# CPCLAB-UNIPI/MPC-code

Measured on NVIDIA B200. Metric: batched MPC steps/sec (Ex_NMPC CSTR, N=50, FP64), higher is better.
Workload: dtype f64

## Files before the change

mpc-code_b200/csrc/mpcb_api.cu:

```cuda
#include <cuda_runtime.h>
#include <stdio.h>
#include <string.h>
#include <stdlib.h>
#include <string>
#include <utility>
#include <vector>
#include "mpcb.h"
#include "mpcb_target.cuh"

#define MPCB_NKERNELS 8
enum { KC_OCP_INIT = 0, KC_OCP_EVAL = 1, KC_OCP_KKT = 2, KC_OCP_TRIAL = 3, KC_OCP_ACCEPT = 4, KC_TARGET = 5, KC_ESTIMATE = 6, KC_OTHER = 7 };

#ifndef MPCB_EVAL_BLOCK
#define MPCB_EVAL_BLOCK 128
#endif
#ifndef MPCB_EVAL_MINBLOCKS
#define MPCB_EVAL_MINBLOCKS 2
#endif

#ifndef MPCB_FLOPS_TABLE
#define MPCB_FLOPS_TABLE
#endif

#if MPCB_HAS_OCP
struct OcpArgs {
    int B;
    const double* par; double* w; double* ws; InstState* st;
    unsigned long long* counters;
    OcpShared S;
};

__device__ __forceinline__ OcpInst ocp_view(const OcpArgs& a, int inst) {
    return ocp_inst(a.ws + (size_t)inst * OcpLayout::total, a.w + (size_t)inst * NW, a.par + (size_t)inst * NPAR, a.st + inst);
}

__global__ void __launch_bounds__(128) k_ocp_init(OcpArgs a) {
    const int tid = blockIdx.x * blockDim.x + threadIdx.x;
    const int inst = tid / (NH + 1), k = tid % (NH + 1);
    if (inst >= a.B) return;
    OcpInst I = ocp_view(a, inst);
    ocp_init_stage(I, a.S, k);
}

#ifndef MPCB_EVAL_SMEM
#define MPCB_EVAL_SMEM ((EVAL_RK_DOUBLES) > 0 && \
                        ((size_t)(EVAL_RK_DOUBLES) * 8 * MPCB_EVAL_BLOCK + 1024) * MPCB_EVAL_MINBLOCKS <= 232448)
#endif
#define EVAL_SMEM_BYTES (MPCB_EVAL_SMEM ? (size_t)(EVAL_RK_DOUBLES) * 8 * MPCB_EVAL_BLOCK : 0)
#ifdef MPCB_EVAL_MAXNREG
#define EVAL_BOUNDS __maxnreg__(MPCB_EVAL_MAXNREG)
#else
#define EVAL_BOUNDS __launch_bounds__(MPCB_EVAL_BLOCK, MPCB_EVAL_MINBLOCKS)
#endif
__global__ void EVAL_BOUNDS k_ocp_eval(OcpArgs a) {
    extern __shared__ double eval_smem[];
    const int tid = blockIdx.x * blockDim.x + threadIdx.x;
    const int inst = tid / NH, k = tid % NH;
    if (inst >= a.B) return;
    if (a.st[inst].state != ST_EVAL) return;
    if (k == 0) atomicAdd(a.counters, 1ULL);
    OcpInst I = ocp_view(a, inst);
    ocp_eval_stage<MPCB_EVAL_SMEM>(I, a.S, k, RkBuf{eval_smem + threadIdx.x, MPCB_EVAL_BLOCK});
}

#if MPCB_EVAL_FIRST
__global__ void __launch_bounds__(128) k_ocp_eval_first(OcpArgs a) {
    const int tid = blockIdx.x * blockDim.x + threadIdx.x;
    const int inst = tid / NH, k = tid % NH;
    if (inst >= a.B) return;
    if (a.st[inst].state != ST_EVAL) return;
    if (k == 0) atomicAdd(a.counters, 1ULL);
    OcpInst I = ocp_view(a, inst);
    ocp_eval_stage<false, true>(I, a.S, k);
}
#endif

#ifndef MPCB_TGT_BLOCK
#define MPCB_TGT_BLOCK 64
#endif
#ifndef KKT_WARPS
#define KKT_SCRATCH_BYTES ((int)sizeof(double) * KktScratch::total * (32 / MPCB_KKT_LANES))
#define KKT_WARPS (4 * KKT_SCRATCH_BYTES <= 48 * 1024 ? 4 : (2 * KKT_SCRATCH_BYTES <= 48 * 1024 ? 2 : 1))
#endif
#if MPCB_KKT_LANES > 1
#ifndef MPCB_FUSE_LS
#define MPCB_FUSE_LS 0
#endif
#ifdef MPCB_KKT_MINBLOCKS
#define KKT_BOUNDS __launch_bounds__(32 * KKT_WARPS, MPCB_KKT_MINBLOCKS)
#else
#define KKT_BOUNDS __launch_bounds__(32 * KKT_WARPS)
#endif
__global__ void KKT_BOUNDS k_ocp_kkt(OcpArgs a, int* n_active) {
    constexpr int GROUPS = 32 * KKT_WARPS / MPCB_KKT_LANES;
    __shared__ __align__(16) double scratch[GROUPS][KktScratch::total];
    const int inst = (blockIdx.x * blockDim.x + threadIdx.x) / MPCB_KKT_LANES;
    if (inst >= a.B) return;
    if (a.st[inst].state != ST_EVAL) return;
    OcpInst I = ocp_view(a, inst);
    ocp_kkt(I, a.S, scratch[threadIdx.x / MPCB_KKT_LANES]);
#if MPCB_FUSE_LS
    const int lane = threadIdx.x & 31;
    volatile int* state = &a.st[inst].state;
    while (*state == ST_LS) {
        if (lane == 0) atomicAdd(a.counters + 1, 1ULL);
        for (int k = lane; k < NH; k += 32) ocp_trial_stage(I, a.S, k);
        __syncwarp();
        ocp_accept(I, a.S);
    }
    if (n_active && lane == 0 && *state != ST_DONE) atomicAdd(n_active, 1);
#else
    (void)n_active;
#endif
}
#define KKT_GRID(B) nblk((long)(B) * MPCB_KKT_LANES, 32 * KKT_WARPS), 32 * KKT_WARPS
#else
#define MPCB_FUSE_LS 0
__global__ void __launch_bounds__(32) k_ocp_kkt(OcpArgs a, int* n_active) {
    (void)n_active;
    const int inst = blockIdx.x * blockDim.x + threadIdx.x;
    if (inst >= a.B) return;
    if (a.st[inst].state != ST_EVAL) return;
    double scratch[KktScratch::total];
    OcpInst I = ocp_view(a, inst);
    ocp_kkt(I, a.S, scratch);
}
#define KKT_GRID(B) nblk((long)(B), 32), 32
#endif

__global__ void __launch_bounds__(128) k_ocp_trial(OcpArgs a) {
    const int tid = blockIdx.x * blockDim.x + threadIdx.x;
    const int inst = tid / NH, k = tid % NH;
    if (inst >= a.B) return;
    if (a.st[inst].state != ST_LS) return;
    if (k == 0) atomicAdd(a.counters + 1, 1ULL);
    OcpInst I = ocp_view(a, inst);
    ocp_trial_stage(I, a.S, k);
}

__global__ void __launch_bounds__(32 * KKT_WARPS) k_ocp_accept(OcpArgs a, int* n_active) {
    const int inst = (blockIdx.x * blockDim.x + threadIdx.x) >> 5;
    if (inst >= a.B) return;
    if (a.st[inst].state == ST_LS) {
        OcpInst I = ocp_view(a, inst);
        ocp_accept(I, a.S);
    }
    if (n_active && (threadIdx.x & 31) == 0 && a.st[inst].state != ST_DONE) atomicAdd(n_active, 1);
}

__global__ void k_ocp_cond(cudaGraphConditionalHandle handle, int* n_active, unsigned long long* ctr, int max_ticks, int ticks) {
    const int active = *n_active;
    *n_active = 0;
    const unsigned long long t = (ctr[0] += (unsigned long long)ticks);
    ctr[1] += (unsigned long long)ticks;
    cudaGraphSetConditional(handle, (active > 0 && t < (unsigned long long)max_ticks) ? 1u : 0u);
}

__global__ void k_ocp_output(OcpArgs a, double* f, int* status, int* iters) {
    const int tid = blockIdx.x * blockDim.x + threadIdx.x;
    const int inst = tid / (NH + 1), k = tid % (NH + 1);
    if (inst >= a.B) return;
    OcpInst I = ocp_view(a, inst);
    ocp_export_stage(I, k);
    if (k == 0) { f[inst] = a.st[inst].fval; status[inst] = a.st[inst].status; iters[inst] = a.st[inst].iter; }
}

__global__ void EVAL_BOUNDS k_stage_derivs(int B, const double* par, const double* w, const double* lam,
                                                      double* A, double* Bm, double* c, double* H) {
    extern __shared__ double eval_smem[];
    const int tid = blockIdx.x * blockDim.x + threadIdx.x;
    const int inst = tid / NH, k = tid % NH;
    if (inst >= B) return;
    const double* wi = w + (size_t)inst * NW; const double* pi = par + (size_t)inst * NPAR;
    double x[NX], u[NU], l[NX], d[ND + 1], px[NPX + 1], py[NPY + 1], t0;
    for (int i = 0; i < NX; ++i) { x[i] = wi[k * NZ + i]; l[i] = lam[((size_t)inst * NH + k) * NX + i]; }
    for (int i = 0; i < NU; ++i) u[i] = wi[k * NZ + NX + i];
    stage_params(pi, k, d, px, py, &t0);
    double xn[NX], Al[NX * NX], Bl[NX * NU], Hp[NZP];
    for (int i = 0; i < NZP; ++i) Hp[i] = 0.0;
    dyn_full<(MPCB_EVAL_SMEM && MPCB_DYN_RK4 && !MPCB_CONTFORM)>(x, u, d, px, t0, l, xn, Al, Bl, Hp, RkBuf{eval_smem + threadIdx.x, MPCB_EVAL_BLOCK});
    const size_t s = (size_t)inst * NH + k;
    for (int i = 0; i < NX * NX; ++i) A[s * NX * NX + i] = Al[i];
    for (int i = 0; i < NX * NU; ++i) Bm[s * NX * NU + i] = Bl[i];
    for (int i = 0; i < NX; ++i) c[s * NX + i] = xn[i] - wi[(k + 1) * NZ + i];
    for (int i = 0; i < NZP; ++i) H[s * NZP + i] = Hp[i];
}
#endif

#if MPCB_HAS_TARGET
__global__ void __launch_bounds__(64) k_target(int B, const double* par, double* w, double* f, int* status, int* iters,
                                               TgtShared S) {
    const int inst = blockIdx.x * blockDim.x + threadIdx.x;
    if (inst >= B) return;
    tgt_solve_regular(par + (size_t)inst * MPCB_NPARSS, w + (size_t)inst * NWS, f + inst, status + inst, iters + inst, S);
}
__global__ void __launch_bounds__(64) k_target_resto(int B, const double* par, double* w, double* f, int* status, int* iters,
                                                     TgtShared S) {
    const int inst = blockIdx.x * blockDim.x + threadIdx.x;
    if (inst >= B) return;
    tgt_solve_resto(par + (size_t)inst * MPCB_NPARSS, w + (size_t)inst * NWS, f + inst, status + inst, iters + inst, S);
}
#endif

__global__ void __launch_bounds__(64) k_estimate(int B, int est_type, const double* y, const double* u, const double* t,
                                                 const double* px, const double* py, double* xi, double* P, EstShared E) {
    const int inst = blockIdx.x * blockDim.x + threadIdx.x;
    if (inst >= B) return;
    est_update(est_type, y + (size_t)inst * NY, u + (size_t)inst * NU, t[inst], px + (size_t)inst * NPX,
               py + (size_t)inst * NPY, xi + (size_t)inst * NXI, P + (size_t)inst * NXI * NXI, E);
}

__global__ void k_model_output(int B, const double* x, const double* u, const double* d, const double* t,
                               const double* py, double* y) {
    const int inst = blockIdx.x * blockDim.x + threadIdx.x;
    if (inst >= B) return;
    double xl[NX], ul[NU], dl[ND + 1], pl[NPY + 1], yl[NY], tt = t[inst];
    for (int i = 0; i < NX; ++i) xl[i] = x[(size_t)inst * NX + i];
    for (int i = 0; i < NU; ++i) ul[i] = u[(size_t)inst * NU + i];
    for (int i = 0; i < ND; ++i) dl[i] = d[(size_t)inst * ND + i];
    for (int i = 0; i < NPY; ++i) pl[i] = py[(size_t)inst * NPY + i];
    mdl_fy(xl, ul, dl, &tt, pl, yl);
    for (int i = 0; i < NY; ++i) y[(size_t)inst * NY + i] = yl[i];
}

__global__ void k_model_step(int B, const double* x, const double* u, const double* d, const double* t,
                             const double* px, double* xn) {
    const int inst = blockIdx.x * blockDim.x + threadIdx.x;
    if (inst >= B) return;
    double xl[NX], ul[NU], dl[ND + 1], pl[NPX + 1], xo[NX];
    for (int i = 0; i < NX; ++i) xl[i] = x[(size_t)inst * NX + i];
    for (int i = 0; i < NU; ++i) ul[i] = u[(size_t)inst * NU + i];
    for (int i = 0; i < ND; ++i) dl[i] = d[(size_t)inst * ND + i];
    for (int i = 0; i < NPX; ++i) pl[i] = px[(size_t)inst * NPX + i];
    dyn_value(xl, ul, dl, pl, t[inst], xo);
    for (int i = 0; i < NX; ++i) xn[(size_t)inst * NX + i] = xo[i];
}

#if !MPCB_PLANT_NOMINAL
__global__ void k_plant_meas(int B, const double* x, const double* u, const double* t, const double* pyp,
                             const double* pymp, const double* noise, double* y) {
    const int inst = blockIdx.x * blockDim.x + threadIdx.x;
    if (inst >= B) return;
    double yl[NY];
    plant_meas(x + (size_t)inst * MPCB_NXP, u + (size_t)inst * NU, t[inst], pyp + (size_t)inst * MPCB_NPYP,
               pymp + (size_t)inst * MPCB_NPYP, yl);
    for (int i = 0; i < NY; ++i) y[(size_t)inst * NY + i] = yl[i] + (noise ? noise[(size_t)inst * NY + i] : 0.0);
}
__global__ void k_plant_step(int B, double* x, const double* u, const double* t, const double* pxp, const double* pxmp) {
    const int inst = blockIdx.x * blockDim.x + threadIdx.x;
    if (inst >= B) return;
    plant_step(x + (size_t)inst * MPCB_NXP, u + (size_t)inst * NU, t[inst], pxp + (size_t)inst * MPCB_NPXP,
               pxmp + (size_t)inst * MPCB_NPXP);
}
#endif


#if MPCB_HAS_OCP && MPCB_HAS_TARGET
struct LoopState {
    double *xi, *P, *u, *us, *xs, *wguess, *wopt, *x0m, *u0, *parss, *wss, *par, *w, *px0, *py0, *fss;
    int *dyn_status, *ss_status, *ss_iters;
};

__global__ void k_step_params(int B, const double* px, const double* py, LoopState L) {
    const int inst = blockIdx.x * blockDim.x + threadIdx.x;
    if (inst >= B) return;
    for (int i = 0; i < NPX; ++i) L.px0[(size_t)inst * NPX + i] = px ? px[(size_t)inst * NPX * NH + i] : 0.0;
    for (int i = 0; i < NPY; ++i) L.py0[(size_t)inst * NPY + i] = py ? py[(size_t)inst * NPY * NH + i] : 0.0;
}

__global__ void k_step_pre(int B, const double* t, const double* sp, LoopState L, double* xhat_out, double* dhat_out) {
    const int inst = blockIdx.x * blockDim.x + threadIdx.x;
    if (inst >= B) return;
    const double* xi = L.xi + (size_t)inst * NXI;
    double* ps = L.parss + (size_t)inst * MPCB_NPARSS;
    for (int i = 0; i < NX; ++i) xhat_out[(size_t)inst * NX + i] = xi[i];
    double d[ND + 1];
    for (int i = 0; i < ND; ++i) { d[i] = (NXI > NX) ? xi[NX + i] : 0.0; dhat_out[(size_t)inst * ND + i] = d[i]; }
    const double* spi = sp + (size_t)inst * (NU + NY + NX);
    for (int i = 0; i < NU; ++i) ps[MPCB_OFFSS_USP + i] = spi[i];
    for (int i = 0; i < NY; ++i) ps[MPCB_OFFSS_YSP + i] = spi[NU + i];
    for (int i = 0; i < NX; ++i) ps[MPCB_OFFSS_XSP + i] = spi[NU + NY + i];
    for (int i = 0; i < ND; ++i) ps[MPCB_OFFSS_D + i] = d[i];
    for (int i = 0; i < NU; ++i) ps[MPCB_OFFSS_USPREV + i] = L.us[(size_t)inst * NU + i];
    for (int i = 0; i < NY * NU; ++i) ps[MPCB_OFFSS_LAM + i] = 0.0;
    ps[MPCB_OFFSS_T] = t[inst];
    double py[NPY + 1];
    for (int i = 0; i < NPX; ++i) ps[MPCB_OFFSS_PX + i] = L.px0[(size_t)inst * NPX + i];
    for (int i = 0; i < NPY; ++i) { py[i] = L.py0[(size_t)inst * NPY + i]; ps[MPCB_OFFSS_PY + i] = py[i]; }
    double* wg = L.wss + (size_t)inst * NWS;
    double x0[NX], u0[NU], y0[NY], tt = t[inst];
    for (int i = 0; i < NX; ++i) { x0[i] = L.x0m[(size_t)inst * NX + i]; wg[i] = x0[i]; }
    for (int i = 0; i < NU; ++i) { u0[i] = L.u0[(size_t)inst * NU + i]; wg[NX + i] = u0[i]; }
    mdl_fy(x0, u0, d, &tt, py, y0);
    for (int i = 0; i < NY; ++i) wg[NZ + i] = y0[i];
}

__global__ void k_step_mid(int B, int first, const double* t, const double* px, const double* py, LoopState L,
                           double* xs_out, double* us_out) {
    const int inst = (blockIdx.x * blockDim.x + threadIdx.x) >> 5, lane = threadIdx.x & 31;
    if (inst >= B) return;
    double* xs = L.xs + (size_t)inst * NX; double* us = L.us + (size_t)inst * NU;
    const double* wss = L.wss + (size_t)inst * NWS;
    const bool ss_ok = L.ss_status[inst] != 2;
    double xs_prev[NX], us_prev[NU], xs_new[NX], us_new[NU];
    for (int i = 0; i < NX; ++i) { xs_prev[i] = xs[i]; xs_new[i] = ss_ok ? wss[i] : xs_prev[i]; }
    for (int i = 0; i < NU; ++i) { us_prev[i] = us[i]; us_new[i] = ss_ok ? wss[NX + i] : us_prev[i]; }
    __syncwarp();
    const double* xi = L.xi + (size_t)inst * NXI;
    double* pr = L.par + (size_t)inst * NPAR;
    if (lane == 0) {
        for (int i = 0; i < NX; ++i) { xs[i] = xs_new[i]; xs_out[(size_t)inst * NX + i] = xs_new[i]; }
        for (int i = 0; i < NU; ++i) { us[i] = us_new[i]; us_out[(size_t)inst * NU + i] = us_new[i]; }
        for (int i = 0; i < NX; ++i) { pr[MPCB_OFF_X0 + i] = xi[i]; pr[MPCB_OFF_XS + i] = xs_new[i]; }
        for (int i = 0; i < NU; ++i) { pr[MPCB_OFF_US + i] = us_new[i]; pr[MPCB_OFF_UM1 + i] = L.u[(size_t)inst * NU + i]; }
        for (int i = 0; i < ND; ++i) pr[MPCB_OFF_D + i] = (NXI > NX) ? xi[NX + i] : 0.0;
        pr[MPCB_OFF_T] = t[inst];
        for (int i = 0; i < NY * NU; ++i) pr[MPCB_OFF_LAM + i] = 0.0;
    }
    for (int i = lane; i < NPX * NH; i += 32) pr[MPCB_OFF_PX + i] = px ? px[(size_t)inst * NPX * NH + i] : 0.0;
    for (int i = lane; i < NPY * NH; i += 32) pr[MPCB_OFF_PY + i] = py ? py[(size_t)inst * NPY * NH + i] : 0.0;
    double* wg = L.wguess + (size_t)inst * NW; double* w = L.w + (size_t)inst * NW;
    const double* wo = L.wopt + (size_t)inst * NW;
    const bool shift = !first && L.dyn_status[inst] != 2 && L.dyn_status[inst] != -13;
    for (int i = lane; i < NW; i += 32) {
        double v;
        if (first) {
            const int r = i % NZ;
            v = (r < NX) ? L.x0m[(size_t)inst * NX + r] : L.u0[(size_t)inst * NU + r - NX];
        } else if (shift) {
            if (i < NW - NZ) v = wo[NZ + i];
            else {
                v = 0.0;
#pragma unroll
                for (int j = 0; j < NU; ++j) if (i == NW - NZ + j) v = us_prev[j];
#pragma unroll
                for (int j = 0; j < NX; ++j) if (i == NW - NX + j) v = xs_prev[j];
            }
        } else {
            v = wg[i];
        }
        wg[i] = v; w[i] = v;
    }
}

__global__ void k_step_post(int B, const double* t, const int* status, LoopState L, double* u_out, int hold_failed) {
    const int inst = (blockIdx.x * blockDim.x + threadIdx.x) >> 5, lane = threadIdx.x & 31;
    if (inst >= B) return;
    double* xi = L.xi + (size_t)inst * NXI; double* u = L.u + (size_t)inst * NU;
    const double* w = L.w + (size_t)inst * NW;
    int st = status[inst];
    if (hold_failed && st < 0 && st != -13) st = 2;
    if (lane == 0) L.dyn_status[inst] = st;
    if (st == -13) {
        for (int i = lane; i < NU; i += 32) u_out[(size_t)inst * NU + i] = u[i];
    } else if (st != 2) {
        double* wo = L.wopt + (size_t)inst * NW;
        for (int i = lane; i < NW; i += 32) wo[i] = w[i];
        for (int i = lane; i < NU; i += 32) { const double v = w[NX + i]; u[i] = v; u_out[(size_t)inst * NU + i] = v; }
        for (int i = lane; i < NX; i += 32) xi[i] = w[NZ + i];
    } else if (lane == 0) {
        double x[NX], ul[NU], d[ND + 1], pxl[NPX + 1], xn[NX];
        for (int i = 0; i < NX; ++i) x[i] = xi[i];
        for (int i = 0; i < NU; ++i) { ul[i] = u[i]; u_out[(size_t)inst * NU + i] = ul[i]; }
        for (int i = 0; i < ND; ++i) d[i] = (NXI > NX) ? xi[NX + i] : 0.0;
        for (int i = 0; i < NPX; ++i) pxl[i] = L.px0[(size_t)inst * NPX + i];
        dyn_value(x, ul, d, pxl, t[inst], xn);
        for (int i = 0; i < NX; ++i) xi[i] = xn[i];
    }
}
#endif

struct mpcb_ctx {
    int B, device;
    mpcb_opts_t opts_ss, opts_dyn;
    std::string err;
    double *ws, *lbx, *ubx, *lbg, *ubg, *ss_lbx, *ss_ubx, *Qkf, *Rkf, *Kest, *dmin, *dmax;
    InstState* st;
    int* n_active; int* h_active;
    int have_dbounds, last_launches, last_ticks;
    cudaGraph_t og_graph; cudaGraphExec_t og_exec;
    const void* og_key[5]; mpcb_opts_t og_opts; int og_valid;
    double* stage_mem; int* stage_imem;
    unsigned long long* tick_ctr;
    long host_launches; int host_loop; cudaStream_t last_stream;
    int hold_failed;
    double* loop_mem; int* loop_imem; int loop_first;
#if MPCB_HAS_OCP && MPCB_HAS_TARGET
    LoopState L;
#endif
    int profile;
    unsigned long long* counters;
    double kernel_ms[MPCB_NKERNELS]; long kernel_launches[MPCB_NKERNELS];
    unsigned long long eval_instances, trial_instances;
    std::vector<cudaEvent_t> ev_pool;
    std::vector<std::pair<int, int>> ev_pending;
    int ngroups;
    std::vector<struct StepGroup*> groups;
    cudaEvent_t ev_in;
};

struct StepGroup { mpcb_ctx* c; int b0, nb; cudaStream_t s; cudaEvent_t done; };

static IpmOpts to_ipm(const mpcb_opts_t& o) {
    IpmOpts r;
    r.max_iter = o.max_iter; r.tol = o.tol; r.mu_init = o.mu_init; r.bound_relax = o.bound_relax_factor;
    r.bound_push = o.bound_push; r.acceptable_tol = o.acceptable_tol;
    r.honor_original_bounds = o.honor_original_bounds; r.acceptable_iter = o.acceptable_iter;
    return r;
}

static int fail(mpcb_ctx* h, const char* what, cudaError_t e) {
    if (h) h->err = std::string(what) + ": " + cudaGetErrorString(e);
    return -1;
}
#define CK(call) do { cudaError_t e_ = (call); if (e_ != cudaSuccess) return fail(h, #call, e_); } while (0)

struct Prof {
    mpcb_ctx* h; cudaStream_t s; int kc; int idx;
    Prof(mpcb_ctx* h_, cudaStream_t s_, int kc_) : h(h_), s(s_), kc(kc_), idx(-1) {
        if (!h->profile) return;
        idx = (int)h->ev_pending.size() * 2;
        while ((int)h->ev_pool.size() < idx + 2) { cudaEvent_t e; cudaEventCreate(&e); h->ev_pool.push_back(e); }
        cudaEventRecord(h->ev_pool[idx], s);
    }
    ~Prof() {
        h->kernel_launches[kc] += 1;
        if (idx < 0) return;
        cudaEventRecord(h->ev_pool[idx + 1], s);
        h->ev_pending.push_back(std::make_pair(kc, idx));
    }
};
static void prof_collect(mpcb_ctx* h) {
    for (auto& p : h->ev_pending) {
        float ms = 0.f;
        if (cudaEventElapsedTime(&ms, h->ev_pool[p.second], h->ev_pool[p.second + 1]) == cudaSuccess) h->kernel_ms[p.first] += ms;
    }
    h->ev_pending.clear();
}

__global__ void k_dfma_peak(double* out, int iters) {
    double a0 = threadIdx.x * 1e-9, a1 = a0 + 1, a2 = a0 + 2, a3 = a0 + 3, a4 = a0 + 4, a5 = a0 + 5, a6 = a0 + 6, a7 = a0 + 7;
    const double b = 1.0000001, c = 1e-9;
    for (int i = 0; i < iters; ++i) {
        a0 = fma(a0, b, c); a1 = fma(a1, b, c); a2 = fma(a2, b, c); a3 = fma(a3, b, c);
        a4 = fma(a4, b, c); a5 = fma(a5, b, c); a6 = fma(a6, b, c); a7 = fma(a7, b, c);
    }
    out[blockIdx.x * blockDim.x + threadIdx.x] = a0 + a1 + a2 + a3 + a4 + a5 + a6 + a7;
}

extern "C" {

int mpcb_abi_version(void) { return MPCB_ABI_VERSION; }

void mpcb_default_opts(mpcb_opts_t* o) {
    o->max_iter = 100; o->tol = 1e-8; o->mu_init = 0.1; o->bound_relax_factor = 1e-8;
    o->honor_original_bounds = 0; o->bound_push = 1e-2; o->acceptable_tol = 1e-6; o->acceptable_iter = 15;
}

int mpcb_get_dims(mpcb_dims_t* d) {
    memset(d, 0, sizeof(*d));
    d->nx = NX; d->nu = NU; d->ny = NY; d->nd = ND; d->npx = NPX; d->npy = NPY;
    d->nxp = MPCB_NXP; d->npxp = MPCB_NPXP; d->npyp = MPCB_NPYP; d->nxi = NXI; d->N = NH; d->Mx = MX;
#if MPCB_HAS_OCP
    d->nw = NW; d->npar = NPAR; d->ng = NG; d->has_ocp = 1;
#endif
#if MPCB_HAS_TARGET
    d->nwss = NWS; d->nparss = MPCB_NPARSS; d->has_target = 1;
#endif
    return 0;
}

long mpcb_model_flops(const char* name) {
    static const struct { const char* n; long f; } table[] = { MPCB_FLOPS_TABLE {nullptr, 0} };
    for (int i = 0; table[i].n; ++i) if (!strcmp(table[i].n, name)) return table[i].f;
    return -1;
}

int mpcb_create(int batch, const mpcb_opts_t* oss, const mpcb_opts_t* odyn, mpcb_handle_t* out) {
    mpcb_ctx* h = new mpcb_ctx();
    h->B = batch; h->have_dbounds = 0; h->last_launches = 0; h->last_ticks = 0;
    h->og_graph = nullptr; h->og_exec = nullptr; h->og_valid = 0; h->tick_ctr = nullptr; h->host_launches = 0; h->last_stream = nullptr;
    h->stage_mem = nullptr; h->stage_imem = nullptr; h->hold_failed = 0;
    { const char* e = getenv("MPCB_HOST_LOOP"); h->host_loop = (e && e[0] == '1') ? 1 : 0; }
    mpcb_default_opts(&h->opts_ss); mpcb_default_opts(&h->opts_dyn);
    if (oss) h->opts_ss = *oss;
    if (odyn) h->opts_dyn = *odyn;
    *out = h;
    if (batch <= 0) { h->err = "batch must be positive"; return -2; }
    CK(cudaGetDevice(&h->device));
    h->ws = nullptr; h->st = nullptr; h->lbx = h->ubx = h->lbg = h->ubg = nullptr;
#if MPCB_HAS_OCP
    CK(cudaMalloc(&h->ws, sizeof(double) * (size_t)batch * OcpLayout::total));
    CK(cudaMemset(h->ws, 0, sizeof(double) * (size_t)batch * OcpLayout::total));
    CK(cudaMalloc(&h->st, sizeof(InstState) * (size_t)batch));
    CK(cudaMalloc(&h->lbx, sizeof(double) * NWI)); CK(cudaMalloc(&h->ubx, sizeof(double) * NWI));
    CK(cudaMalloc(&h->lbg, sizeof(double) * (NH * NGS))); CK(cudaMalloc(&h->ubg, sizeof(double) * (NH * NGS)));
    if (EVAL_SMEM_BYTES > 0) {
        CK(cudaFuncSetAttribute(k_ocp_eval, cudaFuncAttributeMaxDynamicSharedMemorySize, (int)EVAL_SMEM_BYTES));
        CK(cudaFuncSetAttribute(k_stage_derivs, cudaFuncAttributeMaxDynamicSharedMemorySize, (int)EVAL_SMEM_BYTES));
    }
#endif
    h->ss_lbx = h->ss_ubx = nullptr;
#if MPCB_HAS_TARGET
    CK(cudaMalloc(&h->ss_lbx, sizeof(double) * NWS)); CK(cudaMalloc(&h->ss_ubx, sizeof(double) * NWS));
#endif
    CK(cudaMalloc(&h->Qkf, sizeof(double) * NXI * NXI)); CK(cudaMalloc(&h->Rkf, sizeof(double) * NY * NY));
    CK(cudaMalloc(&h->Kest, sizeof(double) * NXI * NY));
    CK(cudaMalloc(&h->dmin, sizeof(double) * (ND + 1))); CK(cudaMalloc(&h->dmax, sizeof(double) * (ND + 1)));
    CK(cudaMemset(h->Qkf, 0, sizeof(double) * NXI * NXI)); CK(cudaMemset(h->Rkf, 0, sizeof(double) * NY * NY));
    CK(cudaMemset(h->Kest, 0, sizeof(double) * NXI * NY));
    CK(cudaMalloc(&h->n_active, sizeof(int)));
    CK(cudaMemset(h->n_active, 0, sizeof(int)));
    CK(cudaMallocHost(&h->h_active, sizeof(int)));
    CK(cudaMalloc(&h->tick_ctr, 2 * sizeof(unsigned long long)));
    CK(cudaMemset(h->tick_ctr, 0, 2 * sizeof(unsigned long long)));
    CK(cudaMalloc(&h->counters, 2 * sizeof(unsigned long long)));
    CK(cudaMemset(h->counters, 0, 2 * sizeof(unsigned long long)));
    h->loop_mem = nullptr; h->loop_imem = nullptr; h->loop_first = 1;
    h->profile = 0; h->eval_instances = h->trial_instances = 0;
    h->ngroups = 1; h->ev_in = nullptr;
    for (int i = 0; i < MPCB_NKERNELS; ++i) { h->kernel_ms[i] = 0.0; h->kernel_launches[i] = 0; }
    return 0;
}

static void groups_teardown(mpcb_ctx* h);

static void ocp_graph_drop(mpcb_ctx* h) {
    if (h->og_exec) cudaGraphExecDestroy(h->og_exec);
    if (h->og_graph) cudaGraphDestroy(h->og_graph);
    h->og_exec = nullptr; h->og_graph = nullptr; h->og_valid = 0;
}

int mpcb_destroy(mpcb_handle_t h) {
    if (!h) return 0;
    cudaDeviceSynchronize();
    groups_teardown(h);
    ocp_graph_drop(h);
    cudaFree(h->tick_ctr); cudaFree(h->stage_mem); cudaFree(h->stage_imem);
    if (h->ev_in) cudaEventDestroy(h->ev_in);
    cudaFree(h->ws); cudaFree(h->st); cudaFree(h->lbx); cudaFree(h->ubx); cudaFree(h->lbg); cudaFree(h->ubg);
    cudaFree(h->ss_lbx); cudaFree(h->ss_ubx); cudaFree(h->Qkf); cudaFree(h->Rkf); cudaFree(h->Kest);
    cudaFree(h->dmin); cudaFree(h->dmax); cudaFree(h->n_active); cudaFreeHost(h->h_active); cudaFree(h->counters);
    for (auto e : h->ev_pool) cudaEventDestroy(e);
    cudaFree(h->loop_mem); cudaFree(h->loop_imem);
    delete h;
    return 0;
}

const char* mpcb_last_error(mpcb_handle_t h) { return h ? h->err.c_str() : "null handle"; }

int mpcb_set_const(mpcb_handle_t h, const char* name, const double* p, int n) {
#if MPCB_HAS_OCP
    if (!strcmp(name, "ocp_lbx") || !strcmp(name, "ocp_ubx")) {
        if (n != NW) { h->err = std::string("mpcb_set_const: wrong length for ") + name; return -2; }
        const bool lower = !strcmp(name, "ocp_lbx");
        std::vector<double> tmp(NWI, lower ? -INFINITY : INFINITY);
        for (int k = 0; k <= NH; ++k) {
            for (int i = 0; i < NX; ++i) tmp[k * NZA + i] = p[k * NZ + i];
            if (k < NH) for (int i = 0; i < NU; ++i) tmp[k * NZA + NXA + i] = p[k * NZ + NX + i];
        }
        CK(cudaMemcpy(lower ? h->lbx : h->ubx, tmp.data(), sizeof(double) * NWI, cudaMemcpyHostToDevice));
        return 0;
    }
#endif
    struct { const char* nm; double* dst; int len; } tab[] = {
#if MPCB_HAS_OCP
        {"ocp_lbg", h->lbg, NH * NG}, {"ocp_ubg", h->ubg, NH * NG},
#endif
#if MPCB_HAS_TARGET
        {"ss_lbx", h->ss_lbx, NWS}, {"ss_ubx", h->ss_ubx, NWS},
#endif
        {"Q_kf", h->Qkf, NXI * NXI}, {"R_kf", h->Rkf, NY * NY}, {"K_est", h->Kest, NXI * NY},
        {"dmin", h->dmin, ND}, {"dmax", h->dmax, ND},
    };
    for (auto& e : tab) {
        if (strcmp(e.nm, name)) continue;
        if (n != e.len) { h->err = std::string("mpcb_set_const: wrong length for ") + name; return -2; }
        if (n > 0) CK(cudaMemcpy(e.dst, p, sizeof(double) * n, cudaMemcpyHostToDevice));
        if (!strcmp(name, "dmax")) h->have_dbounds = 1;
        return 0;
    }
    h->err = std::string("mpcb_set_const: unknown name ") + name;
    return -2;
}

static inline int nblk(long n, int bs) { return (int)((n + bs - 1) / bs); }

static bool same_opts(const mpcb_opts_t& a, const mpcb_opts_t& b) {
    return a.max_iter == b.max_iter && a.tol == b.tol && a.mu_init == b.mu_init && a.bound_relax_factor == b.bound_relax_factor &&
           a.honor_original_bounds == b.honor_original_bounds && a.bound_push == b.bound_push &&
           a.acceptable_tol == b.acceptable_tol && a.acceptable_iter == b.acceptable_iter;
}

#if MPCB_HAS_OCP
#define TICK_KERNELS (MPCB_FUSE_LS ? 2 : 4)
static int add_tick(mpcb_ctx* h, cudaGraph_t g, cudaGraphNode_t* dep, int ndep, OcpArgs& a, int* n_active, cudaGraphNode_t* last,
                    bool first = false) {
    const int bs = 128;
    const long nst = (long)h->B * NH;
    cudaKernelNodeParams kp; memset(&kp, 0, sizeof(kp));
    void* args1[] = {&a};
    cudaGraphNode_t n_eval;
    kp.kernelParams = args1;
    kp.func = (void*)k_ocp_eval; kp.gridDim = dim3(nblk(nst, MPCB_EVAL_BLOCK)); kp.blockDim = dim3(MPCB_EVAL_BLOCK);
    kp.sharedMemBytes = (unsigned)EVAL_SMEM_BYTES;
#if MPCB_EVAL_FIRST
    if (first) { kp.func = (void*)k_ocp_eval_first; kp.gridDim = dim3(nblk(nst, 128)); kp.blockDim = dim3(128); kp.sharedMemBytes = 0; }
#else
    (void)first;
#endif
    CK(cudaGraphAddKernelNode(&n_eval, g, dep, ndep, &kp));
    kp.sharedMemBytes = 0;
    { dim3 gk(1), bk(1); auto set = [&](int gx, int bx) { gk = dim3(gx); bk = dim3(bx); }; set(KKT_GRID(h->B));
      kp.func = (void*)k_ocp_kkt; kp.gridDim = gk; kp.blockDim = bk; }
    void* args2[] = {&a, &n_active};
    kp.kernelParams = args2;
#if MPCB_FUSE_LS
    (void)bs;
    CK(cudaGraphAddKernelNode(last, g, &n_eval, 1, &kp));
#else
    cudaGraphNode_t n_kkt, n_trial;
    CK(cudaGraphAddKernelNode(&n_kkt, g, &n_eval, 1, &kp));
    kp.kernelParams = args1;
    kp.func = (void*)k_ocp_trial; kp.gridDim = dim3(nblk(nst, bs)); kp.blockDim = dim3(bs);
    CK(cudaGraphAddKernelNode(&n_trial, g, &n_kkt, 1, &kp));
    kp.func = (void*)k_ocp_accept; kp.gridDim = dim3(nblk((long)h->B * 32, 32 * KKT_WARPS)); kp.blockDim = dim3(32 * KKT_WARPS);
    kp.kernelParams = args2;
    CK(cudaGraphAddKernelNode(last, g, &n_trial, 1, &kp));
#endif
    return 0;
}

static int ocp_graph_build(mpcb_ctx* h, const OcpArgs& a_in, double* f, int* status, int* iters) {
    ocp_graph_drop(h);
    OcpArgs a = a_in;
    const int bs = 128;
    int max_ticks = (h->opts_dyn.max_iter + 2) * 8;
    int unroll = 10;
    { const char* e = getenv("MPCB_GRAPH_UNROLL"); if (e) unroll = atoi(e); }
    if (unroll < 0) unroll = 0;
    if (unroll > max_ticks) unroll = max_ticks;
    CK(cudaGraphCreate(&h->og_graph, 0));
    cudaGraph_t g = h->og_graph;
    cudaGraphNode_t n_ms1, n_ms2, n_init, n_while, n_out, prev;
    cudaMemsetParams ms; memset(&ms, 0, sizeof(ms));
    ms.dst = h->n_active; ms.value = 0; ms.elementSize = 4; ms.width = 1; ms.height = 1; ms.pitch = 4;
    CK(cudaGraphAddMemsetNode(&n_ms1, g, nullptr, 0, &ms));
    ms.dst = h->tick_ctr; ms.width = 2;
    CK(cudaGraphAddMemsetNode(&n_ms2, g, nullptr, 0, &ms));
    cudaKernelNodeParams kp; memset(&kp, 0, sizeof(kp));
    void* args1[] = {&a};
    kp.func = (void*)k_ocp_init; kp.gridDim = dim3(nblk((long)h->B * (NH + 1), bs)); kp.blockDim = dim3(bs); kp.kernelParams = args1;
    cudaGraphNode_t dep0[] = {n_ms1, n_ms2};
    CK(cudaGraphAddKernelNode(&n_init, g, dep0, 2, &kp));
    prev = n_init;
    int* n_active = h->n_active; int* no_count = nullptr;
    for (int t = 0; t < unroll; ++t) {
        cudaGraphNode_t last;
        int rc = add_tick(h, g, &prev, 1, a, (t == unroll - 1) ? n_active : no_count, &last, t == 0);
        if (rc) return rc;
        prev = last;
    }
    cudaGraphConditionalHandle handle;
    CK(cudaGraphConditionalHandleCreate(&handle, g, 1, cudaGraphCondAssignDefault));
    unsigned long long* ctr = h->tick_ctr;
    if (unroll > 0) {
        cudaGraphNode_t n_c0;
        void* args3[] = {&handle, &n_active, &ctr, &max_ticks, &unroll};
        kp.func = (void*)k_ocp_cond; kp.gridDim = dim3(1); kp.blockDim = dim3(1); kp.kernelParams = args3; kp.sharedMemBytes = 0;
        CK(cudaGraphAddKernelNode(&n_c0, g, &prev, 1, &kp));
        prev = n_c0;
    }
    cudaGraphNodeParams cp = { cudaGraphNodeTypeConditional };
    cp.conditional.handle = handle; cp.conditional.type = cudaGraphCondTypeWhile; cp.conditional.size = 1;
    CK(cudaGraphAddNode(&n_while, g, &prev, 1, &cp));
    cudaGraph_t body = cp.conditional.phGraph_out[0];
    {
        cudaGraphNode_t last, n_cond;
        int rc = add_tick(h, body, nullptr, 0, a, n_active, &last);
        if (rc) return rc;
        int one = 1;
        void* args3[] = {&handle, &n_active, &ctr, &max_ticks, &one};
        kp.func = (void*)k_ocp_cond; kp.gridDim = dim3(1); kp.blockDim = dim3(1); kp.kernelParams = args3; kp.sharedMemBytes = 0;
        CK(cudaGraphAddKernelNode(&n_cond, body, &last, 1, &kp));
    }
    void* args4[] = {&a, &f, &status, &iters};
    kp.func = (void*)k_ocp_output; kp.gridDim = dim3(nblk((long)h->B * (NH + 1), 128)); kp.blockDim = dim3(128); kp.kernelParams = args4;
    CK(cudaGraphAddKernelNode(&n_out, g, &n_while, 1, &kp));
    CK(cudaGraphInstantiate(&h->og_exec, g, 0));
    h->og_key[0] = a.par; h->og_key[1] = a.w; h->og_key[2] = f; h->og_key[3] = status; h->og_key[4] = iters;
    h->og_opts = h->opts_dyn; h->og_valid = 1;
    return 0;
}

static int ocp_host_loop(mpcb_ctx* h, OcpArgs& a, double* f, int* status, int* iters, cudaStream_t s) {
    const int bs = 128;
    const long nst = (long)h->B * NH;
    int launches = 0, ticks = 0;
    CK(cudaMemsetAsync(h->n_active, 0, sizeof(int), s));
    { Prof p(h, s, KC_OCP_INIT); k_ocp_init<<<nblk((long)h->B * (NH + 1), bs), bs, 0, s>>>(a); } launches++;
    const int max_ticks = (h->opts_dyn.max_iter + 2) * 8;
    const int check_every = 2;
    while (ticks < max_ticks) {
        for (int c = 0; c < check_every; ++c) {
#if MPCB_EVAL_FIRST
            if (ticks == 0) { Prof p(h, s, KC_OCP_EVAL); k_ocp_eval_first<<<nblk(nst, 128), 128, 0, s>>>(a); }
            else
#endif
            { Prof p(h, s, KC_OCP_EVAL); k_ocp_eval<<<nblk(nst, MPCB_EVAL_BLOCK), MPCB_EVAL_BLOCK, EVAL_SMEM_BYTES, s>>>(a); }
#if MPCB_FUSE_LS
            if (c == check_every - 1) CK(cudaMemsetAsync(h->n_active, 0, sizeof(int), s));
            { Prof p(h, s, KC_OCP_KKT); k_ocp_kkt<<<KKT_GRID(h->B), 0, s>>>(a, h->n_active); }
#else
            { Prof p(h, s, KC_OCP_KKT); k_ocp_kkt<<<KKT_GRID(h->B), 0, s>>>(a, nullptr); }
            { Prof p(h, s, KC_OCP_TRIAL); k_ocp_trial<<<nblk(nst, bs), bs, 0, s>>>(a); }
            if (c == check_every - 1) CK(cudaMemsetAsync(h->n_active, 0, sizeof(int), s));
            { Prof p(h, s, KC_OCP_ACCEPT); k_ocp_accept<<<nblk((long)h->B * 32, 32 * KKT_WARPS), 32 * KKT_WARPS, 0, s>>>(a, h->n_active); }
#endif
            launches += TICK_KERNELS; ticks++;
        }
        CK(cudaMemcpyAsync(h->h_active, h->n_active, sizeof(int), cudaMemcpyDeviceToHost, s));
        CK(cudaStreamSynchronize(s));
        prof_collect(h);
        if (*h->h_active == 0) break;
    }
    CK(cudaMemsetAsync(h->n_active, 0, sizeof(int), s));
    { Prof p(h, s, KC_OTHER); k_ocp_output<<<nblk((long)h->B * (NH + 1), 128), 128, 0, s>>>(a, f, status, iters); } launches++;
    CK(cudaGetLastError());
    if (h->profile) {
        unsigned long long cnt[2];
        CK(cudaMemcpyAsync(cnt, h->counters, sizeof(cnt), cudaMemcpyDeviceToHost, s));
        CK(cudaStreamSynchronize(s));
        prof_collect(h);
        h->eval_instances = cnt[0]; h->trial_instances = cnt[1];
    }
    h->host_launches += launches;
    h->last_launches = launches; h->last_ticks = ticks;
    return 0;
}
#endif

int mpcb_ocp(mpcb_handle_t h, const double* par, double* w, double* f, int* status, int* iters, void* stream) {
#if MPCB_HAS_OCP
    cudaStream_t s = (cudaStream_t)stream;
    OcpArgs a;
    a.B = h->B; a.par = par; a.w = w; a.ws = h->ws; a.st = h->st; a.counters = h->counters;
    a.S.lbx = h->lbx; a.S.ubx = h->ubx; a.S.lbg = h->lbg; a.S.ubg = h->ubg; a.S.o = to_ipm(h->opts_dyn);
    h->last_stream = s;
    if (h->profile || h->host_loop) return ocp_host_loop(h, a, f, status, iters, s);
    const void* key[5] = {par, w, f, status, iters};
    const bool moved = h->og_valid && memcmp(key, h->og_key, sizeof(key)) != 0;
    const size_t B = (size_t)h->B;
    if (moved && !h->stage_mem) {
        CK(cudaMalloc(&h->stage_mem, sizeof(double) * B * (NPAR + NW + 1)));
        CK(cudaMalloc(&h->stage_imem, sizeof(int) * B * 2));
    }
    const bool staged = h->stage_mem != nullptr;
    double* sp_ = h->stage_mem; double* sw_ = sp_ + B * NPAR; double* sf_ = sw_ + B * NW;
    int* sst_ = h->stage_imem; int* sit_ = sst_ + B;
    if (staged) {
        CK(cudaMemcpyAsync(sp_, par, sizeof(double) * B * NPAR, cudaMemcpyDeviceToDevice, s));
        CK(cudaMemcpyAsync(sw_, w, sizeof(double) * B * NW, cudaMemcpyDeviceToDevice, s));
        a.par = sp_; a.w = sw_;
        key[0] = sp_; key[1] = sw_; key[2] = sf_; key[3] = sst_; key[4] = sit_;
    }
    if (!h->og_valid || memcmp(key, h->og_key, sizeof(key)) || !same_opts(h->og_opts, h->opts_dyn)) {
        int rc = staged ? ocp_graph_build(h, a, sf_, sst_, sit_) : ocp_graph_build(h, a, f, status, iters);
        if (rc) return rc;
    }
    CK(cudaGraphLaunch(h->og_exec, s));
    if (staged) {
        CK(cudaMemcpyAsync(w, sw_, sizeof(double) * B * NW, cudaMemcpyDeviceToDevice, s));
        CK(cudaMemcpyAsync(f, sf_, sizeof(double) * B, cudaMemcpyDeviceToDevice, s));
        CK(cudaMemcpyAsync(status, sst_, sizeof(int) * B, cudaMemcpyDeviceToDevice, s));
        CK(cudaMemcpyAsync(iters, sit_, sizeof(int) * B, cudaMemcpyDeviceToDevice, s));
    }
    h->host_launches += 2;
    h->last_launches = -1; h->last_ticks = -1;
    return 0;
#else
    h->err = "library built without the OCP"; return -3;
#endif
}

int mpcb_stage_derivs(mpcb_handle_t h, const double* par, const double* w, const double* lam,
                      double* A, double* Bm, double* c, double* H, void* stream) {
#if MPCB_HAS_OCP
    h->host_launches += 1;
    { Prof p(h, (cudaStream_t)stream, KC_OTHER); k_stage_derivs<<<nblk((long)h->B * NH, MPCB_EVAL_BLOCK), MPCB_EVAL_BLOCK, EVAL_SMEM_BYTES, (cudaStream_t)stream>>>(h->B, par, w, lam, A, Bm, c, H); }
    CK(cudaGetLastError());
    h->last_launches = 1;
    return 0;
#else
    h->err = "library built without the OCP"; return -3;
#endif
}

int mpcb_target(mpcb_handle_t h, const double* par_ss, double* wss, double* fss, int* status, int* iters, void* stream) {
#if MPCB_HAS_TARGET
    TgtShared S; S.lbx = h->ss_lbx; S.ubx = h->ss_ubx; S.o = to_ipm(h->opts_ss);
    { Prof p(h, (cudaStream_t)stream, KC_TARGET); k_target<<<nblk(h->B, MPCB_TGT_BLOCK), MPCB_TGT_BLOCK, 0, (cudaStream_t)stream>>>(h->B, par_ss, wss, fss, status, iters, S); }
#if !MPCB_DENSE_SH
    { Prof p(h, (cudaStream_t)stream, KC_TARGET); k_target_resto<<<nblk(h->B, MPCB_TGT_BLOCK), MPCB_TGT_BLOCK, 0, (cudaStream_t)stream>>>(h->B, par_ss, wss, fss, status, iters, S); }
    h->host_launches += 1;
#endif
    CK(cudaGetLastError());
    if (h->profile) { CK(cudaStreamSynchronize((cudaStream_t)stream)); prof_collect(h); }
    h->host_launches += 1; h->last_stream = (cudaStream_t)stream;
    h->last_launches = 1; h->last_ticks = 1;
    return 0;
#else
    h->err = "library built without the target problem"; return -3;
#endif
}

int mpcb_estimate(mpcb_handle_t h, int est_type, const double* y, const double* u, const double* t, const double* px,
                  const double* py, double* xi, double* P, void* stream) {
    EstShared E; E.Q = h->Qkf; E.R = h->Rkf; E.K = h->Kest; E.dmin = h->dmin; E.dmax = h->dmax; E.has_dbounds = h->have_dbounds;
    { Prof p(h, (cudaStream_t)stream, KC_ESTIMATE); k_estimate<<<nblk(h->B, 64), 64, 0, (cudaStream_t)stream>>>(h->B, est_type, y, u, t, px, py, xi, P, E); }
    CK(cudaGetLastError());
    h->host_launches += 1;
    return 0;
}

int mpcb_model_output(mpcb_handle_t h, const double* x, const double* u, const double* d, const double* t,
                      const double* py, double* y, void* stream) {
    h->kernel_launches[KC_OTHER] += 1; h->host_launches += 1;
    k_model_output<<<nblk(h->B, 128), 128, 0, (cudaStream_t)stream>>>(h->B, x, u, d, t, py, y);
    CK(cudaGetLastError());
    return 0;
}

int mpcb_model_step(mpcb_handle_t h, const double* x, const double* u, const double* d, const double* t,
                    const double* px, double* xn, void* stream) {
    h->kernel_launches[KC_OTHER] += 1; h->host_launches += 1;
    k_model_step<<<nblk(h->B, 128), 128, 0, (cudaStream_t)stream>>>(h->B, x, u, d, t, px, xn);
    CK(cudaGetLastError());
    return 0;
}

int mpcb_plant_meas(mpcb_handle_t h, const double* x, const double* u, const double* t, const double* pyp,
                    const double* pymp, const double* noise, double* y, void* stream) {
#if !MPCB_PLANT_NOMINAL
    h->kernel_launches[KC_OTHER] += 1; h->host_launches += 1;
    k_plant_meas<<<nblk(h->B, 128), 128, 0, (cudaStream_t)stream>>>(h->B, x, u, t, pyp, pymp, noise, y);
    CK(cudaGetLastError());
    return 0;
#else
    h->err = "nominal plant: use mpcb_model_output (MPC_code.py:531-532)"; return -3;
#endif
}

int mpcb_plant_step(mpcb_handle_t h, double* x, const double* u, const double* t, const double* pxp,
                    const double* pxmp, void* stream) {
#if !MPCB_PLANT_NOMINAL
    h->kernel_launches[KC_OTHER] += 1; h->host_launches += 1;
    k_plant_step<<<nblk(h->B, 128), 128, 0, (cudaStream_t)stream>>>(h->B, x, u, t, pxp, pxmp);
    CK(cudaGetLastError());
    return 0;
#else
    h->err = "nominal plant: use mpcb_model_step (MPC_code.py:813-814)"; return -3;
#endif
}

int mpcb_set_profiling(mpcb_handle_t h, int on) {
    h->profile = on ? 1 : 0;
    if (on) while (h->ev_pool.size() < 2 * 1024) { cudaEvent_t e; if (cudaEventCreate(&e) != cudaSuccess) break; h->ev_pool.push_back(e); }
    for (int i = 0; i < MPCB_NKERNELS; ++i) { h->kernel_ms[i] = 0.0; h->kernel_launches[i] = 0; }
    h->eval_instances = h->trial_instances = 0;
    CK(cudaDeviceSynchronize());
    CK(cudaMemset(h->counters, 0, 2 * sizeof(unsigned long long)));
    for (StepGroup* g : h->groups) {
        mpcb_ctx* c = g->c;
        c->profile = h->profile;
        for (int i = 0; i < MPCB_NKERNELS; ++i) { c->kernel_ms[i] = 0.0; c->kernel_launches[i] = 0; }
        c->eval_instances = c->trial_instances = 0;
        CK(cudaMemset(c->counters, 0, 2 * sizeof(unsigned long long)));
        if (on) while (c->ev_pool.size() < 2 * 1024) { cudaEvent_t e; if (cudaEventCreate(&e) != cudaSuccess) break; c->ev_pool.push_back(e); }
    }
    return 0;
}

int mpcb_get_profile(mpcb_handle_t h, double* kernel_ms, long* kernel_launches, unsigned long long* instance_counts) {
    for (int i = 0; i < MPCB_NKERNELS; ++i) { kernel_ms[i] = h->kernel_ms[i]; kernel_launches[i] = h->kernel_launches[i]; }
    instance_counts[0] = h->eval_instances; instance_counts[1] = h->trial_instances;
    for (StepGroup* g : h->groups) {
        for (int i = 0; i < MPCB_NKERNELS; ++i) { kernel_ms[i] += g->c->kernel_ms[i]; kernel_launches[i] += g->c->kernel_launches[i]; }
        instance_counts[0] += g->c->eval_instances; instance_counts[1] += g->c->trial_instances;
    }
    return 0;
}

int mpcb_dfma_peak(int iters, double* tflops) {
    const int blocks = 148 * 16, threads = 256;
    double* out = nullptr;
    if (cudaMalloc(&out, sizeof(double) * blocks * threads) != cudaSuccess) return -1;
    cudaEvent_t e0, e1; cudaEventCreate(&e0); cudaEventCreate(&e1);
    k_dfma_peak<<<blocks, threads>>>(out, 1000);
    double best = 0.0;
    for (int rep = 0; rep < 5; ++rep) {
        cudaEventRecord(e0);
        k_dfma_peak<<<blocks, threads>>>(out, iters);
        cudaEventRecord(e1);
        if (cudaEventSynchronize(e1) != cudaSuccess) { cudaFree(out); return -1; }
        float ms = 0.f; cudaEventElapsedTime(&ms, e0, e1);
        const double fl = 2.0 * 8.0 * (double)iters * blocks * threads;
        if (ms > 0.f && fl / (ms * 1e-3) / 1e12 > best) best = fl / (ms * 1e-3) / 1e12;
    }
    cudaEventDestroy(e0); cudaEventDestroy(e1); cudaFree(out);
    *tflops = best;
    return 0;
}

int mpcb_loop_reset(mpcb_handle_t h, const double* x0_m, const double* u0, const double* dhat0, const double* P0) {
#if MPCB_HAS_OCP && MPCB_HAS_TARGET
    const size_t B = (size_t)h->B;
    if (!h->loop_mem) {
        const size_t n = B * (NXI + NXI * NXI + 3 * NU + 2 * NX + 3 * NW + MPCB_NPARSS + NWS + NPAR + NPX + NPY + 1);
        CK(cudaMalloc(&h->loop_mem, sizeof(double) * n));
        CK(cudaMalloc(&h->loop_imem, sizeof(int) * 3 * B));
        double* p = h->loop_mem;
        LoopState& L = h->L;
        L.xi = p; p += B * NXI; L.P = p; p += B * NXI * NXI; L.u = p; p += B * NU; L.us = p; p += B * NU; L.u0 = p; p += B * NU;
        L.xs = p; p += B * NX; L.x0m = p; p += B * NX; L.wguess = p; p += B * NW; L.wopt = p; p += B * NW; L.w = p; p += B * NW;
        L.parss = p; p += B * MPCB_NPARSS; L.wss = p; p += B * NWS; L.par = p; p += B * NPAR; L.px0 = p; p += B * NPX;
        L.py0 = p; p += B * NPY; L.fss = p; p += B;
        L.dyn_status = h->loop_imem; L.ss_status = h->loop_imem + B; L.ss_iters = h->loop_imem + 2 * B;
    }
    LoopState& L = h->L;
    CK(cudaMemset(h->loop_mem, 0, sizeof(double) * B * (NXI + NXI * NXI)));
    CK(cudaMemset(h->loop_imem, 0, sizeof(int) * 3 * B));
    CK(cudaMemcpy2D(L.xi, sizeof(double) * NXI, x0_m, sizeof(double) * NX, sizeof(double) * NX, B, cudaMemcpyDeviceToDevice));
    if (NXI > NX && dhat0)
        CK(cudaMemcpy2D(L.xi + NX, sizeof(double) * NXI, dhat0, sizeof(double) * ND, sizeof(double) * ND, B, cudaMemcpyDeviceToDevice));
    if (P0) CK(cudaMemcpy(L.P, P0, sizeof(double) * B * NXI * NXI, cudaMemcpyDeviceToDevice));
    CK(cudaMemcpy(L.x0m, x0_m, sizeof(double) * B * NX, cudaMemcpyDeviceToDevice));
    CK(cudaMemcpy(L.xs, x0_m, sizeof(double) * B * NX, cudaMemcpyDeviceToDevice));
    CK(cudaMemcpy(L.u0, u0, sizeof(double) * B * NU, cudaMemcpyDeviceToDevice));
    CK(cudaMemcpy(L.u, u0, sizeof(double) * B * NU, cudaMemcpyDeviceToDevice));
    CK(cudaMemcpy(L.us, u0, sizeof(double) * B * NU, cudaMemcpyDeviceToDevice));
    h->loop_first = 1;
    return 0;
#else
    h->err = "library built without OCP/target"; return -3;
#endif
}

int mpcb_loop_get(mpcb_handle_t h, double* xi, double* P, double* u, void* stream) {
#if MPCB_HAS_OCP && MPCB_HAS_TARGET
    if (!h->loop_mem) { h->err = "mpcb_loop_reset has not been called"; return -2; }
    cudaStream_t s = (cudaStream_t)stream;
    const size_t B = (size_t)h->B;
    if (xi) CK(cudaMemcpyAsync(xi, h->L.xi, sizeof(double) * B * NXI, cudaMemcpyDeviceToDevice, s));
    if (P) CK(cudaMemcpyAsync(P, h->L.P, sizeof(double) * B * NXI * NXI, cudaMemcpyDeviceToDevice, s));
    if (u) CK(cudaMemcpyAsync(u, h->L.u, sizeof(double) * B * NU, cudaMemcpyDeviceToDevice, s));
    return 0;
#else
    h->err = "library built without OCP/target"; return -3;
#endif
}

static int step_impl(mpcb_ctx* h, int est_type, const double* y_meas, const double* t, const double* sp, const double* px,
              const double* py, double* u_out, double* xhat_out, double* dhat_out, double* xs_out, double* us_out,
              double* f_dyn, int* status_dyn, int* iters_dyn, int* status_ss, void* stream) {
#if MPCB_HAS_OCP && MPCB_HAS_TARGET
    if (!h->loop_mem) { h->err = "mpcb_loop_reset has not been called"; return -2; }
    cudaStream_t s = (cudaStream_t)stream;
    LoopState& L = h->L;
    const int B = h->B, g = nblk(B, 128);
    k_step_params<<<g, 128, 0, s>>>(B, px, py, L);
    int rc = mpcb_estimate(h, est_type, y_meas, L.u, t, L.px0, L.py0, L.xi, L.P, s);
    if (rc) return rc;
    k_step_pre<<<g, 128, 0, s>>>(B, t, sp, L, xhat_out, dhat_out);
    rc = mpcb_target(h, L.parss, L.wss, L.fss, L.ss_status, L.ss_iters, s);
    if (rc) return rc;
    k_step_mid<<<nblk((long)B * 32, 128), 128, 0, s>>>(B, h->loop_first, t, px, py, L, xs_out, us_out);
    rc = mpcb_ocp(h, L.par, L.w, f_dyn, status_dyn, iters_dyn, s);
    if (rc) return rc;
    k_step_post<<<nblk((long)B * 32, 128), 128, 0, s>>>(B, t, status_dyn, L, u_out, h->hold_failed);
    if (status_ss) CK(cudaMemcpyAsync(status_ss, L.ss_status, sizeof(int) * B, cudaMemcpyDeviceToDevice, s));
    CK(cudaGetLastError());
    h->kernel_launches[KC_OTHER] += 4; h->host_launches += 4;
    h->loop_first = 0;
    return 0;
#else
    h->err = "library built without OCP/target"; return -3;
#endif
}


#if MPCB_HAS_OCP && MPCB_HAS_TARGET
static int groups_setup(mpcb_ctx* h) {
    groups_teardown(h);
    const int G = h->ngroups, B = h->B, per = (B + G - 1) / G;
    if (!h->ev_in) CK(cudaEventCreateWithFlags(&h->ev_in, cudaEventDisableTiming));
    for (int b0 = 0; b0 < B; b0 += per) {
        StepGroup* g = new StepGroup();
        g->b0 = b0; g->nb = (b0 + per <= B) ? per : B - b0;
        mpcb_ctx* c = new mpcb_ctx();
        c->device = h->device; c->opts_ss = h->opts_ss; c->opts_dyn = h->opts_dyn; c->have_dbounds = h->have_dbounds;
        c->lbx = h->lbx; c->ubx = h->ubx; c->lbg = h->lbg; c->ubg = h->ubg; c->ss_lbx = h->ss_lbx; c->ss_ubx = h->ss_ubx;
        c->Qkf = h->Qkf; c->Rkf = h->Rkf; c->Kest = h->Kest; c->dmin = h->dmin; c->dmax = h->dmax;
        c->loop_mem = h->loop_mem; c->loop_imem = h->loop_imem; c->loop_first = h->loop_first;
        c->profile = h->profile; c->host_loop = h->host_loop; c->ngroups = 1; c->ev_in = nullptr; c->hold_failed = h->hold_failed;
        c->og_graph = nullptr; c->og_exec = nullptr; c->og_valid = 0; c->host_launches = 0; c->last_stream = nullptr;
        c->eval_instances = c->trial_instances = 0;
        for (int i = 0; i < MPCB_NKERNELS; ++i) { c->kernel_ms[i] = 0.0; c->kernel_launches[i] = 0; }
        c->B = g->nb;
        c->ws = h->ws + (size_t)b0 * OcpLayout::total; c->st = h->st + b0;
        if (cudaMalloc(&c->n_active, sizeof(int)) != cudaSuccess || cudaMallocHost(&c->h_active, sizeof(int)) != cudaSuccess ||
            cudaMalloc(&c->counters, 2 * sizeof(unsigned long long)) != cudaSuccess ||
            cudaMalloc(&c->tick_ctr, 2 * sizeof(unsigned long long)) != cudaSuccess) { h->err = "group allocation failed"; return -1; }
        cudaMemset(c->counters, 0, 2 * sizeof(unsigned long long));
        cudaMemset(c->tick_ctr, 0, 2 * sizeof(unsigned long long));
        cudaMemset(c->n_active, 0, sizeof(int));
        const size_t o = (size_t)b0;
        LoopState& L = c->L; const LoopState& P = h->L;
        L.xi = P.xi + o * NXI; L.P = P.P + o * NXI * NXI; L.u = P.u + o * NU; L.us = P.us + o * NU; L.u0 = P.u0 + o * NU;
        L.xs = P.xs + o * NX; L.x0m = P.x0m + o * NX; L.wguess = P.wguess + o * NW; L.wopt = P.wopt + o * NW; L.w = P.w + o * NW;
        L.parss = P.parss + o * MPCB_NPARSS; L.wss = P.wss + o * NWS; L.par = P.par + o * NPAR; L.px0 = P.px0 + o * NPX;
        L.py0 = P.py0 + o * NPY; L.fss = P.fss + o;
        L.dyn_status = P.dyn_status + o; L.ss_status = P.ss_status + o; L.ss_iters = P.ss_iters + o;
        g->c = c;
        if (cudaStreamCreateWithFlags(&g->s, cudaStreamNonBlocking) != cudaSuccess ||
            cudaEventCreateWithFlags(&g->done, cudaEventDisableTiming) != cudaSuccess) { h->err = "group stream creation failed"; return -1; }
        h->groups.push_back(g);
    }
    return 0;
}
#endif

static void groups_teardown(mpcb_ctx* h) {
#if MPCB_HAS_OCP && MPCB_HAS_TARGET
    for (StepGroup* g : h->groups) {
        cudaStreamSynchronize(g->s);
        h->host_launches += g->c->host_launches;
        unsigned long long ctr[2] = {0, 0};
        cudaMemcpy(ctr, g->c->tick_ctr, sizeof(ctr), cudaMemcpyDeviceToHost);
        h->host_launches += TICK_KERNELS * (long)ctr[1];
        cudaStreamDestroy(g->s); cudaEventDestroy(g->done);
        ocp_graph_drop(g->c);
        cudaFree(g->c->n_active); cudaFreeHost(g->c->h_active); cudaFree(g->c->counters); cudaFree(g->c->tick_ctr);
        for (auto e : g->c->ev_pool) cudaEventDestroy(e);
        delete g->c; delete g;
    }
#endif
    h->groups.clear();
}

int mpcb_set_policy(mpcb_handle_t h, int hold_failed) { h->hold_failed = hold_failed ? 1 : 0; return 0; }

int mpcb_set_groups(mpcb_handle_t h, int n) {
    if (n < 1 || n > h->B) { h->err = "mpcb_set_groups: need 1 <= n <= batch"; return -2; }
    if (n != h->ngroups) { groups_teardown(h); h->ngroups = n; }
    return 0;
}

int mpcb_step(mpcb_handle_t h, int est_type, const double* y_meas, const double* t, const double* sp, const double* px,
              const double* py, double* u_out, double* xhat_out, double* dhat_out, double* xs_out, double* us_out,
              double* f_dyn, int* status_dyn, int* iters_dyn, int* status_ss, void* stream) {
#if MPCB_HAS_OCP && MPCB_HAS_TARGET
    h->last_stream = (cudaStream_t)stream;
    if (h->ngroups <= 1)
        return step_impl(h, est_type, y_meas, t, sp, px, py, u_out, xhat_out, dhat_out, xs_out, us_out, f_dyn, status_dyn,
                         iters_dyn, status_ss, stream);
    if (!h->loop_mem) { h->err = "mpcb_loop_reset has not been called"; return -2; }
    if (h->groups.empty()) { int rc = groups_setup(h); if (rc) return rc; }
    CK(cudaEventRecord(h->ev_in, (cudaStream_t)stream));
    int rc = 0;
    for (StepGroup* g : h->groups) {
        const size_t o = (size_t)g->b0;
        mpcb_ctx* c = g->c;
        c->opts_ss = h->opts_ss; c->opts_dyn = h->opts_dyn; c->have_dbounds = h->have_dbounds; c->loop_first = h->loop_first;
        c->profile = h->profile; c->hold_failed = h->hold_failed;
        CK(cudaStreamWaitEvent(g->s, h->ev_in, 0));
        const int r = step_impl(c, est_type, y_meas + o * NY, t + o, sp + o * (NU + NY + NX), px ? px + o * NPX * NH : nullptr,
                                py ? py + o * NPY * NH : nullptr, u_out + o * NU, xhat_out + o * NX, dhat_out + o * ND,
                                xs_out + o * NX, us_out + o * NU, f_dyn + o, status_dyn + o, iters_dyn + o,
                                status_ss ? status_ss + o : nullptr, g->s);
        if (r && !rc) { rc = r; h->err = c->err; }
        CK(cudaEventRecord(g->done, g->s));
        CK(cudaStreamWaitEvent((cudaStream_t)stream, g->done, 0));
    }
    h->loop_first = 0;
    return rc;
#else
    h->err = "library built without OCP/target"; return -3;
#endif
}

static void read_ticks(mpcb_ctx* h, unsigned long long* last, unsigned long long* total) {
    unsigned long long ctr[2] = {0, 0};
    cudaStreamSynchronize(h->last_stream);
    cudaMemcpy(ctr, h->tick_ctr, sizeof(ctr), cudaMemcpyDeviceToHost);
    *last = ctr[0]; *total = ctr[1];
}

int mpcb_last_ticks(mpcb_handle_t h) {
    if (h->last_ticks >= 0 && h->groups.empty()) return h->last_ticks;
    unsigned long long last = 0, total = 0, worst = 0;
    if (h->groups.empty()) { read_ticks(h, &last, &total); return (int)last; }
    for (StepGroup* g : h->groups) {
        cudaStreamSynchronize(g->s);
        if (g->c->last_ticks >= 0) { worst = worst > (unsigned long long)g->c->last_ticks ? worst : (unsigned long long)g->c->last_ticks; continue; }
        read_ticks(g->c, &last, &total);
        worst = worst > last ? worst : last;
    }
    return (int)worst;
}

long mpcb_total_launches(mpcb_handle_t h) {
    unsigned long long last = 0, total = 0;
    read_ticks(h, &last, &total);
    long n = h->host_launches + TICK_KERNELS * (long)total;
    for (StepGroup* g : h->groups) {
        cudaStreamSynchronize(g->s);
        read_ticks(g->c, &last, &total);
        n += g->c->host_launches + TICK_KERNELS * (long)total;
    }
    return n;
}

int mpcb_last_launches(mpcb_handle_t h) { return h->last_launches; }

}
```

mpc-code_b200/csrc/mpcb_target.cuh:

```cuda
#pragma once
#include "mpcb_ocp.cuh"

#define NWS  MPCB_NWSS
#ifndef MPCB_NGSS
#define MPCB_NGSS 0
#endif
#ifndef MPCB_NHSS
#define MPCB_NHSS 0
#endif
#define NGT  MPCB_NGSS
#define NHT  MPCB_NHSS
#define NOUT (NY + NGT + NHT)
#define NVT  (NWS + NGT)
#define MCS  (NX + NOUT)
#define NKS  (NVT + MCS)
#define NWSP (NWS * (NWS + 1) / 2)

template <int N>
MPCB_HD void bk_factor(double* A, int* ipiv, int* npos, int* nneg, int* nzero) {
    const double alpha = (1.0 + sqrt(17.0)) / 8.0;
    *npos = *nneg = *nzero = 0;
    int k = 0;
    while (k < N) {
        int kstep = 1, kp = k;
        const double absakk = fabs(A[k + N * k]);
        int imax = k; double colmax = 0.0;
        for (int i = k + 1; i < N; ++i) { const double v = fabs(A[i + N * k]); if (v > colmax) { colmax = v; imax = i; } }
        if (fmax(absakk, colmax) == 0.0) {
            *nzero += 1; ipiv[k] = k + 1; k += 1; continue;
        }
        if (absakk >= alpha * colmax) {
            kp = k;
        } else {
            double rowmax = 0.0;
            for (int j = k; j < imax; ++j) rowmax = fmax(rowmax, fabs(A[imax + N * j]));
            for (int i = imax + 1; i < N; ++i) rowmax = fmax(rowmax, fabs(A[i + N * imax]));
            if (absakk >= alpha * colmax * (colmax / rowmax)) kp = k;
            else if (fabs(A[imax + N * imax]) >= alpha * rowmax) kp = imax;
            else { kp = imax; kstep = 2; }
        }
        const int kk = k + kstep - 1;
        if (kp != kk) {
            for (int i = kp + 1; i < N; ++i) { const double t = A[i + N * kk]; A[i + N * kk] = A[i + N * kp]; A[i + N * kp] = t; }
            for (int j = kk + 1; j < kp; ++j) { const double t = A[j + N * kk]; A[j + N * kk] = A[kp + N * j]; A[kp + N * j] = t; }
            { const double t = A[kk + N * kk]; A[kk + N * kk] = A[kp + N * kp]; A[kp + N * kp] = t; }
            if (kstep == 2) { const double t = A[k + 1 + N * k]; A[k + 1 + N * k] = A[kp + N * k]; A[kp + N * k] = t; }
        }
        if (kstep == 1) {
            const double dkk = A[k + N * k];
            if (dkk > 0.0) *npos += 1; else if (dkk < 0.0) *nneg += 1; else *nzero += 1;
            const double r1 = 1.0 / dkk;
            for (int j = k + 1; j < N; ++j) {
                const double ajk = A[j + N * k] * r1;
                for (int i = j; i < N; ++i) A[i + N * j] -= A[i + N * k] * ajk;
            }
            for (int i = k + 1; i < N; ++i) A[i + N * k] *= r1;
            ipiv[k] = kp + 1;
        } else {
            const double a = A[k + N * k], b = A[k + 1 + N * k], c = A[k + 1 + N * (k + 1)];
            const double det = a * c - b * b;
            if (det < 0.0) { *npos += 1; *nneg += 1; }
            else if (det > 0.0) { if (a + c > 0.0) *npos += 2; else *nneg += 2; }
            else *nzero += 1;
            if (k < N - 2) {
                double d21 = b;
                const double d11 = c / d21, d22 = a / d21;
                const double t = 1.0 / (d11 * d22 - 1.0);
                d21 = t / d21;
                for (int j = k + 2; j < N; ++j) {
                    const double wk = d21 * (d11 * A[j + N * k] - A[j + N * (k + 1)]);
                    const double wkp1 = d21 * (d22 * A[j + N * (k + 1)] - A[j + N * k]);
                    for (int i = j; i < N; ++i) A[i + N * j] -= A[i + N * k] * wk + A[i + N * (k + 1)] * wkp1;
                    A[j + N * k] = wk;
                    A[j + N * (k + 1)] = wkp1;
                }
            }
            ipiv[k] = -(kp + 1); ipiv[k + 1] = -(kp + 1);
        }
        k += kstep;
    }
}

template <int N>
MPCB_HD void bk_solve(const double* A, const int* ipiv, double* b) {
    int k = 0;
    while (k < N) {
        if (ipiv[k] > 0) {
            const int kp = ipiv[k] - 1;
            if (kp != k) { const double t = b[k]; b[k] = b[kp]; b[kp] = t; }
            for (int i = k + 1; i < N; ++i) b[i] -= b[k] * A[i + N * k];
            b[k] /= A[k + N * k];
            k += 1;
        } else {
            const int kp = -ipiv[k] - 1;
            if (kp != k + 1) { const double t = b[k + 1]; b[k + 1] = b[kp]; b[kp] = t; }
            for (int i = k + 2; i < N; ++i) b[i] -= b[k] * A[i + N * k] + b[k + 1] * A[i + N * (k + 1)];
            const double akm1k = A[k + 1 + N * k];
            const double akm1 = A[k + N * k] / akm1k, ak = A[k + 1 + N * (k + 1)] / akm1k;
            const double denom = akm1 * ak - 1.0;
            const double bkm1 = b[k] / akm1k, bk = b[k + 1] / akm1k;
            b[k] = (ak * bkm1 - bk) / denom;
            b[k + 1] = (akm1 * bk - bkm1) / denom;
            k += 2;
        }
    }
    k = N - 1;
    while (k >= 0) {
        if (ipiv[k] > 0) {
            double a = b[k];
            for (int i = k + 1; i < N; ++i) a -= A[i + N * k] * b[i];
            b[k] = a;
            const int kp = ipiv[k] - 1;
            if (kp != k) { const double t = b[k]; b[k] = b[kp]; b[kp] = t; }
            k -= 1;
        } else {
            double a = b[k], a1 = b[k - 1];
            for (int i = k + 1; i < N; ++i) { a -= A[i + N * k] * b[i]; a1 -= A[i + N * (k - 1)] * b[i]; }
            b[k] = a; b[k - 1] = a1;
            const int kp = -ipiv[k] - 1;
            if (kp != k) { const double t = b[k]; b[k] = b[kp]; b[kp] = t; }
            k -= 2;
        }
    }
}

#if MPCB_HAS_TARGET
struct TgtShared { const double *lbx, *ubx; IpmOpts o; };

MPCB_HD void tgt_eval(const double* w, const double* par, const double* lam, bool derivs,
                      double* f, double* c, double* grad, double* J , double* Hp ) {
    const double* d = par + MPCB_OFFSS_D; const double* px = par + MPCB_OFFSS_PX;
    const double t0 = par[MPCB_OFFSS_T];
    double dl[ND + 1], pxl[NPX + 1];
    for (int i = 0; i < ND; ++i) dl[i] = d[i];
    for (int i = 0; i < NPX; ++i) pxl[i] = px[i];
    double xn[NX];
    if (!derivs) {
        dyn_value(w, w + NX, dl, pxl, t0, xn);
        for (int i = 0; i < NX; ++i) c[i] = xn[i] - w[i];
        tgt_out(w, par, c + NX);
        for (int i = 0; i < NGT; ++i) c[NX + NY + i] -= w[NWS + i];
        tgt_cost(w, par, f);
        return;
    }
    double A[NX * NX], Bm[NX * NU], Hd[NZP], Hc[NWSP], Ho[NWSP], Jo[NOUT * NWS];
    for (int i = 0; i < NZP; ++i) Hd[i] = 0.0;
    dyn_full(w, w + NX, dl, pxl, t0, lam, xn, A, Bm, Hd);
    for (int i = 0; i < NX; ++i) c[i] = xn[i] - w[i];
    tgt_out_d(w, par, lam + NX, c + NX, Jo, Ho);
    for (int i = 0; i < NGT; ++i) c[NX + NY + i] -= w[NWS + i];
    tgt_cost_d(w, par, f, grad, Hc);
    for (int i = 0; i < NGT; ++i) grad[NWS + i] = 0.0;
    for (int i = 0; i < NWSP; ++i) Hp[i] = Hc[i] + Ho[i];
    for (int i = 0; i < NZP; ++i) Hp[i] += Hd[i];
    for (int j = 0; j < NWS; ++j) {
        for (int i = 0; i < NX; ++i) {
            double v = 0.0;
            if (j < NX) v = A[i + NX * j] - (i == j ? 1.0 : 0.0);
            else if (j < NZ) v = Bm[i + NX * (j - NX)];
            J[i + MCS * j] = v;
        }
        for (int i = 0; i < NOUT; ++i) J[NX + i + MCS * j] = Jo[i + NOUT * j];
    }
    for (int j = 0; j < NGT; ++j)
        for (int i = 0; i < MCS; ++i) J[i + MCS * (NWS + j)] = (i == NX + NY + j) ? -1.0 : 0.0;
}

#define TGT_NEEDS_RESTO 1000
template <bool MPCB_TGT_RESTO>
MPCB_HD void tgt_solve_t(const double* par, double* w_io, double* fout, int* status_out, int* iters_out, const TgtShared& S) {
    const IpmOpts& o = S.o;
    const double rf = o.bound_relax;
    double w[NVT], lo[NVT], hi[NVT]; bool hl[NVT], hu[NVT];
    int nb = 0;
    for (int i = 0; i < NWS; ++i) {
        hl[i] = fin(S.lbx[i]); hu[i] = fin(S.ubx[i]);
        lo[i] = hl[i] ? rlo(S.lbx[i], rf) : S.lbx[i];
        hi[i] = hu[i] ? rhi(S.ubx[i], rf) : S.ubx[i];
        nb += (hl[i] ? 1 : 0) + (hu[i] ? 1 : 0);
        w[i] = push_in(w_io[i], lo[i], hi[i], o.bound_push);
    }
    if (NGT > 0) {
        double f0, c0[MCS];
        for (int i = NWS; i < NVT; ++i) w[i] = 0.0;
        tgt_eval(w, par, nullptr, false, &f0, c0, nullptr, nullptr, nullptr);
        for (int i = NWS; i < NVT; ++i) {
            hl[i] = false; hu[i] = true; lo[i] = -INFINITY; hi[i] = rhi(0.0, rf); nb += 1;
            w[i] = push_in(c0[NX + NY + (i - NWS)], lo[i], hi[i], o.bound_push);
        }
    }
    double y[MCS], zL[NVT], zU[NVT];
    for (int i = 0; i < MCS; ++i) y[i] = 0.0;
    for (int i = 0; i < NVT; ++i) { zL[i] = hl[i] ? 1.0 : 0.0; zU[i] = hu[i] ? 1.0 : 0.0; }
    double mu = o.mu_init, tau = fmax(0.99, 1.0 - mu), dw_last = 0.0, theta0 = -1.0;
    double filt[2 * MPCB_MAXFILT]; int nfilt = 0, acc = 0, it = 0, status = -1;
    bool resto = false; int resto_calls = 0; double theta_entry = 0.0;
    double f = 0.0, c[MCS], grad[NVT], J[MCS * NVT], Hp[NWSP];
    bool evaluate = true;
    while (true) {
        if (evaluate) tgt_eval(w, par, y, true, &f, c, grad, J, Hp);
        evaluate = false;
        if (it == 0 && !resto) {
            double chk = f;
            for (int i = 0; i < MCS; ++i) chk += c[i];
            for (int i = 0; i < NVT; ++i) chk += grad[i];
            if (!(chk == chk) || !fin(chk)) { status = -13; break; }
        }
        double dual = 0.0, prim = 0.0, ysum = 0.0, zsum = 0.0, c0 = 0.0;
        for (int j = 0; j < NVT; ++j) {
            double r = grad[j] - zL[j] + zU[j];
            for (int i = 0; i < MCS; ++i) r += J[i + MCS * j] * y[i];
            dual = fmax(dual, fabs(r));
            zsum += zL[j] + zU[j];
            if (hl[j]) c0 = fmax(c0, fabs((w[j] - lo[j]) * zL[j]));
            if (hu[j]) c0 = fmax(c0, fabs((hi[j] - w[j]) * zU[j]));
        }
        for (int i = 0; i < MCS; ++i) { prim = fmax(prim, fabs(c[i])); ysum += fabs(y[i]); }
        const double sd = fmax(100.0, (ysum + zsum) / (double)(MCS + nb > 0 ? MCS + nb : 1)) / 100.0;
        const double sc = fmax(100.0, zsum / (double)(nb > 0 ? nb : 1)) / 100.0;
        const double E0 = fmax(fmax(dual / sd, prim), c0 / sc);
        if (!(E0 == E0) || !fin(E0)) { status = -13; break; }
        if (!resto) {
            if (E0 <= o.tol && dual <= 1.0 && prim <= 1e-4 && c0 <= 1e-4) { status = 0; break; }
            if (E0 <= o.acceptable_tol && dual <= 1e10 && prim <= 1e-2 && c0 <= 1e-2) {
                if (++acc >= o.acceptable_iter) { status = 1; break; }
            } else acc = 0;
        }
        if (it >= o.max_iter) { status = -1; break; }
        const double mu_min = o.tol / 10.0;
        bool changed = false;
        while (!resto && mu > mu_min) {
            double cm = 0.0;
            for (int j = 0; j < NVT; ++j) {
                if (hl[j]) cm = fmax(cm, fabs((w[j] - lo[j]) * zL[j] - mu));
                if (hu[j]) cm = fmax(cm, fabs((hi[j] - w[j]) * zU[j] - mu));
            }
            if (fmax(fmax(dual / sd, prim), cm / sc) > 10.0 * mu) break;
            mu = fmax(mu_min, fmin(0.2 * mu, pow(mu, 1.5)));
            changed = true;
        }
        if (changed) { tau = fmax(0.99, 1.0 - mu); nfilt = 0; }
        double K[NKS * NKS], rhs[NKS]; int ipiv[NKS];
        double dwreg = 0.0, dcreg = 0.0; bool first = true, ok = false;
        for (int attempt = 0; attempt < 60; ++attempt) {
            for (int i = 0; i < NKS * NKS; ++i) K[i] = 0.0;
            for (int j = 0; j < NVT; ++j) {
                if (j < NWS) for (int i = j; i < NWS; ++i) K[i + NKS * j] = resto ? 0.0 : Hp[tri(i, j)];
                double sig = dwreg;
                if (resto) {
                    const double sc = fmax(1.0, fabs(w[j]));
                    sig += sqrt(mu) / (sc * sc);
                    if (hl[j]) { const double d = w[j] - lo[j]; sig += mu / (d * d); }
                    if (hu[j]) { const double d = hi[j] - w[j]; sig += mu / (d * d); }
                } else {
                    if (hl[j]) sig += zL[j] / (w[j] - lo[j]);
                    if (hu[j]) sig += zU[j] / (hi[j] - w[j]);
                }
                K[j + NKS * j] += sig;
                for (int i = 0; i < MCS; ++i) K[NVT + i + NKS * j] = J[i + MCS * j];
            }
            for (int i = 0; i < MCS; ++i) K[NVT + i + NKS * (NVT + i)] = -dcreg;
            int np_, nn_, nz_;
            bk_factor<NKS>(K, ipiv, &np_, &nn_, &nz_);
            if (np_ == NVT && nn_ == MCS && nz_ == 0) { ok = true; break; }
            if (nz_ > 0) dcreg = 1e-8 * pow(mu, 0.25);
            if (first) { dwreg = (dw_last == 0.0) ? 1e-4 : fmax(1e-20, dw_last / 3.0); first = false; }
            else dwreg *= (dw_last == 0.0) ? 100.0 : 8.0;
            if (dwreg > 1e40) break;
        }
        if (!ok) { status = -3; break; }
        if (dwreg > 0.0) dw_last = dwreg;
        for (int j = 0; j < NVT; ++j) {
            double r = grad[j];
            for (int i = 0; i < MCS; ++i) r += J[i + MCS * j] * y[i];
            if (resto) r = 0.0;
            if (hl[j]) r -= mu / (w[j] - lo[j]);
            if (hu[j]) r += mu / (hi[j] - w[j]);
            rhs[j] = -r;
        }
        for (int i = 0; i < MCS; ++i) rhs[NVT + i] = -c[i];
        bk_solve<NKS>(K, ipiv, rhs);
        double amax = 1.0, az = 1.0, gphid = 0.0, barr = 0.0, theta = 0.0;
        double dzL[NVT], dzU[NVT];
        for (int j = 0; j < NVT; ++j) {
            const double dv = rhs[j];
            gphid += grad[j] * dv;
            dzL[j] = dzU[j] = 0.0;
            if (hl[j]) {
                const double dl = w[j] - lo[j];
                barr += log(dl); gphid -= mu / dl * dv;
                if (dv < 0.0) amax = fmin(amax, -tau * dl / dv);
                dzL[j] = mu / dl - zL[j] - zL[j] / dl * dv;
                if (dzL[j] < 0.0) az = fmin(az, -tau * zL[j] / dzL[j]);
            }
            if (hu[j]) {
                const double du = hi[j] - w[j];
                barr += log(du); gphid += mu / du * dv;
                if (dv > 0.0) amax = fmin(amax, tau * du / dv);
                dzU[j] = mu / du - zU[j] + zU[j] / du * dv;
                if (dzU[j] < 0.0) az = fmin(az, -tau * zU[j] / dzU[j]);
            }
        }
        for (int i = 0; i < MCS; ++i) theta += fabs(c[i]);
        const double phi = f - mu * barr;
        if (theta0 < 0.0) theta0 = theta;
        const double theta_min = 1e-4 * fmax(1.0, theta0), theta_max = 1e4 * fmax(1.0, theta0);
        double amin;
        if (gphid < 0.0 && theta <= theta_min) amin = fmin(1e-5, fmin(1e-8 * theta / (-gphid), pow(theta, 1.1) / pow(-gphid, 2.3)));
        else if (gphid < 0.0) amin = fmin(1e-5, 1e-8 * theta / (-gphid));
        else amin = 1e-5;
        amin *= 0.05;
        double alpha = amax; bool accepted = false, ftype = false;
        double wt[NVT], ft, ct[MCS];
        if (MPCB_TGT_RESTO && resto) {
            double th_t = 0.0;
            while (alpha > 1e-5) {
                for (int j = 0; j < NVT; ++j) wt[j] = w[j] + alpha * rhs[j];
                tgt_eval(wt, par, y, false, &ft, ct, nullptr, nullptr, nullptr);
                th_t = 0.0;
                for (int i = 0; i < MCS; ++i) th_t += fabs(ct[i]);
                if ((th_t == th_t) && fin(th_t) && th_t <= (1.0 - 1e-4 * alpha) * theta) { accepted = true; break; }
                alpha *= 0.5;
            }
            if (!accepted) { status = theta > 1e-4 ? 2 : -2; break; }
            double b_t = 0.0;
            for (int j = 0; j < NVT; ++j) {
                w[j] = wt[j];
                if (hl[j]) { const double d = w[j] - lo[j]; zL[j] = mu / d; b_t += log(d); }
                if (hu[j]) { const double d = hi[j] - w[j]; zU[j] = mu / d; b_t += log(d); }
            }
            for (int i = 0; i < MCS; ++i) y[i] = 0.0;
            const double ph_t = ft - mu * b_t;
            bool leave = th_t <= 0.9 * theta_entry;
            if (leave) for (int i = 0; i < nfilt; ++i) if (th_t >= filt[2 * i] && ph_t >= filt[2 * i + 1]) { leave = false; break; }
            if (leave) resto = false;
            it += 1;
            evaluate = true;
            continue;
        }
        while (alpha >= amin * (1.0 - 1e-12) && alpha > 1e-16) {
            for (int j = 0; j < NVT; ++j) wt[j] = w[j] + alpha * rhs[j];
            tgt_eval(wt, par, y, false, &ft, ct, nullptr, nullptr, nullptr);
            double th_t = 0.0, b_t = 0.0;
            for (int i = 0; i < MCS; ++i) th_t += fabs(ct[i]);
            for (int j = 0; j < NVT; ++j) { if (hl[j]) b_t += log(wt[j] - lo[j]); if (hu[j]) b_t += log(hi[j] - wt[j]); }
            const double ph_t = ft - mu * b_t;
            bool okk = (th_t == th_t) && (ph_t == ph_t) && fin(th_t) && fin(ph_t) && th_t <= theta_max;
            if (okk) for (int i = 0; i < nfilt; ++i) if (th_t >= filt[2 * i] && ph_t >= filt[2 * i + 1]) { okk = false; break; }
            if (okk) {
                const bool sw = gphid < 0.0 && theta <= theta_min && alpha * pow(-gphid, 2.3) > pow(theta, 1.1);
                const double eps = 10.0 * 2.220446049250313e-16 * fabs(phi);
                if (sw) { if (ph_t - phi - eps <= 1e-8 * alpha * gphid) { accepted = true; ftype = true; } }
                else if (th_t <= (1.0 - 1e-5) * theta || ph_t - eps <= phi - 1e-8 * theta) accepted = true;
            }
            if (accepted) break;
            alpha *= 0.5;
        }
        if (!accepted) {
            if (theta < 1e-6 || resto_calls >= 3) { status = theta > 1e-4 ? 2 : -2; break; }
            if (!MPCB_TGT_RESTO) { status = TGT_NEEDS_RESTO; break; }
            if (nfilt < MPCB_MAXFILT) { filt[2 * nfilt] = (1.0 - 1e-5) * theta; filt[2 * nfilt + 1] = phi - 1e-8 * theta; nfilt++; }
            resto = true; resto_calls += 1; theta_entry = theta;
            continue;
        }
        if (!ftype && nfilt < MPCB_MAXFILT) { filt[2 * nfilt] = (1.0 - 1e-5) * theta; filt[2 * nfilt + 1] = phi - 1e-8 * theta; nfilt++; }
        for (int j = 0; j < NVT; ++j) {
            w[j] = wt[j];
            if (hl[j]) { const double dn = w[j] - lo[j]; zL[j] = fmax(fmin(zL[j] + az * dzL[j], 1e10 * mu / dn), mu / (1e10 * dn)); }
            if (hu[j]) { const double dn = hi[j] - w[j]; zU[j] = fmax(fmin(zU[j] + az * dzU[j], 1e10 * mu / dn), mu / (1e10 * dn)); }
        }
        for (int i = 0; i < MCS; ++i) y[i] += alpha * rhs[NVT + i];
        it += 1;
        evaluate = true;
    }
    if (o.honor_original_bounds) {
        for (int j = 0; j < NWS; ++j) w[j] = fmin(fmax(w[j], S.lbx[j]), S.ubx[j]);
        double ct[MCS];
        tgt_eval(w, par, y, false, &f, ct, nullptr, nullptr, nullptr);
    }
    for (int j = 0; j < NWS; ++j) w_io[j] = w[j];
    *fout = f; *status_out = status; *iters_out = it;
}

MPCB_HD void tgt_solve_regular(const double* par, double* w, double* fout, int* status_out, int* iters_out, const TgtShared& S) {
#if MPCB_DENSE_SH
    tgt_solve_t<true>(par, w, fout, status_out, iters_out, S);
#else
    double w0[NWS];
    for (int i = 0; i < NWS; ++i) w0[i] = w[i];
    tgt_solve_t<false>(par, w, fout, status_out, iters_out, S);
    if (*status_out == TGT_NEEDS_RESTO)
        for (int i = 0; i < NWS; ++i) w[i] = w0[i];
#endif
}
MPCB_HD void tgt_solve_resto(const double* par, double* w, double* fout, int* status_out, int* iters_out, const TgtShared& S) {
    if (*status_out == TGT_NEEDS_RESTO) tgt_solve_t<true>(par, w, fout, status_out, iters_out, S);
}
MPCB_HD void tgt_solve(const double* par, double* w, double* fout, int* status_out, int* iters_out, const TgtShared& S) {
    tgt_solve_regular(par, w, fout, status_out, iters_out, S);
    tgt_solve_resto(par, w, fout, status_out, iters_out, S);
}
#endif

struct EstShared { const double *Q, *R, *K, *dmin, *dmax; int has_dbounds; };

MPCB_HD void est_update(int est_type, const double* y_meas, const double* u, double t, const double* px,
                        const double* py, double* xi, double* P, const EstShared& E) {
    double x[NX], d[ND + 1], ul[NU], pxl[NPX + 1], pyl[NPY + 1];
    for (int i = 0; i < NX; ++i) x[i] = xi[i];
    for (int i = 0; i < ND; ++i) d[i] = (NXI > NX) ? xi[NX + i] : 0.0;
    for (int i = 0; i < NU; ++i) ul[i] = u[i];
    for (int i = 0; i < NPX; ++i) pxl[i] = px[i];
    for (int i = 0; i < NPY; ++i) pyl[i] = py[i];
    double yhat[NY], C[NY * NXI], e[NY];
    mdl_fy_xi(x, ul, d, &t, pyl, yhat, C);
    for (int i = 0; i < NY; ++i) e[i] = y_meas[i] - yhat[i];
    if (est_type == 0) {
        for (int i = 0; i < NXI; ++i) {
            double a = xi[i];
            for (int j = 0; j < NY; ++j) a += E.K[i * NY + j] * e[j];
            xi[i] = a;
        }
    } else {
        double PCt[NXI * NY], Sm[NY * NY], L[NY * NY];
        for (int i = 0; i < NXI; ++i)
            for (int j = 0; j < NY; ++j) {
                double a = 0.0;
                for (int l = 0; l < NXI; ++l) a += P[i * NXI + l] * C[j + NY * l];
                PCt[i * NY + j] = a;
            }
        for (int i = 0; i < NY; ++i)
            for (int j = 0; j < NY; ++j) {
                double a = E.R[i * NY + j];
                for (int l = 0; l < NXI; ++l) a += C[i + NY * l] * PCt[l * NY + j];
                Sm[i * NY + j] = a;
            }
        int piv[NY];
        for (int i = 0; i < NY; ++i)
            for (int j = 0; j < NY; ++j) L[i * NY + j] = Sm[j * NY + i];
        for (int c = 0; c < NY; ++c) {
            int pr = c; double best = fabs(L[c * NY + c]);
            for (int i = c + 1; i < NY; ++i) if (fabs(L[i * NY + c]) > best) { best = fabs(L[i * NY + c]); pr = i; }
            piv[c] = pr;
            if (pr != c) for (int j = 0; j < NY; ++j) { double tmp = L[c * NY + j]; L[c * NY + j] = L[pr * NY + j]; L[pr * NY + j] = tmp; }
            double inv = 1.0 / L[c * NY + c];
            for (int i = c + 1; i < NY; ++i) {
                double f = L[i * NY + c] * inv;
                L[i * NY + c] = f;
                for (int j = c + 1; j < NY; ++j) L[i * NY + j] -= f * L[c * NY + j];
            }
        }
        double Kg[NXI * NY];
        for (int r = 0; r < NXI; ++r) {
            double yv[NY];
            for (int i = 0; i < NY; ++i) yv[i] = PCt[r * NY + i];
            for (int c = 0; c < NY; ++c) if (piv[c] != c) { double tmp = yv[c]; yv[c] = yv[piv[c]]; yv[piv[c]] = tmp; }
            for (int i = 1; i < NY; ++i) {
                double a = yv[i];
                for (int l = 0; l < i; ++l) a -= L[i * NY + l] * yv[l];
                yv[i] = a;
            }
            for (int i = NY - 1; i >= 0; --i) {
                double a = yv[i];
                for (int l = i + 1; l < NY; ++l) a -= L[i * NY + l] * yv[l];
                yv[i] = a / L[i * NY + i];
            }
            for (int i = 0; i < NY; ++i) Kg[r * NY + i] = yv[i];
        }
        double CP[NY * NXI], Pc[NXI * NXI];
        for (int i = 0; i < NY; ++i)
            for (int j = 0; j < NXI; ++j) {
                double a = 0.0;
                for (int l = 0; l < NXI; ++l) a += C[i + NY * l] * P[l * NXI + j];
                CP[i * NXI + j] = a;
            }
        for (int i = 0; i < NXI; ++i) {
            double a = xi[i];
            for (int j = 0; j < NY; ++j) a += Kg[i * NY + j] * e[j];
            xi[i] = a;
            for (int j = 0; j < NXI; ++j) {
                double m = P[i * NXI + j];
                for (int l = 0; l < NY; ++l) m -= Kg[i * NY + l] * CP[l * NXI + j];
                Pc[i * NXI + j] = m;
            }
        }
        for (int i = 0; i < NX; ++i) x[i] = xi[i];
        for (int i = 0; i < ND; ++i) d[i] = (NXI > NX) ? xi[NX + i] : 0.0;
        double Axi[NXI * NXI], AP[NXI * NXI];
        dyn_jac_xi(x, ul, d, pxl, t, Axi);
        for (int i = 0; i < NXI; ++i)
            for (int j = 0; j < NXI; ++j) {
                double a = 0.0;
                for (int l = 0; l < NXI; ++l) a += Axi[i * NXI + l] * Pc[l * NXI + j];
                AP[i * NXI + j] = a;
            }
        for (int i = 0; i < NXI; ++i)
            for (int j = 0; j < NXI; ++j) {
                double a = E.Q[i * NXI + j];
                for (int l = 0; l < NXI; ++l) a += AP[i * NXI + l] * Axi[j * NXI + l];
                P[i * NXI + j] = a;
            }
    }
    if (E.has_dbounds && NXI > NX)
        for (int i = 0; i < ND; ++i) xi[NX + i] = fmin(fmax(xi[NX + i], E.dmin[i]), E.dmax[i]);
}

#if !MPCB_PLANT_NOMINAL
MPCB_HD void plant_meas(const double* x, const double* u, double t, const double* pyp, const double* pymp, double* y) {
    double xl[MPCB_NXP], ul[NU], a[MPCB_NPYP + 1], b[MPCB_NPYP + 1];
    for (int i = 0; i < MPCB_NXP; ++i) xl[i] = x[i];
    for (int i = 0; i < NU; ++i) ul[i] = u[i];
    for (int i = 0; i < MPCB_NPYP; ++i) { a[i] = pyp[i]; b[i] = pymp[i]; }
    plt_fy(xl, ul, a, &t, b, y);
}
MPCB_HD void plant_step(double* x, const double* u, double t0, const double* pxp, const double* pxmp) {
    double xc[MPCB_NXP], ul[NU], a[MPCB_NPXP + 1], b[MPCB_NPXP + 1];
    for (int i = 0; i < MPCB_NXP; ++i) xc[i] = x[i];
    for (int i = 0; i < NU; ++i) ul[i] = u[i];
    for (int i = 0; i < MPCB_NPXP; ++i) { a[i] = pxp[i]; b[i] = pxmp[i]; }
#if MPCB_PLANT_RK4
    const double hs = MPCB_HSTEP / MPCB_PMX;
    for (int j = 0; j < MPCB_PMX; ++j) {
        double k1[MPCB_NXP], k2[MPCB_NXP], k3[MPCB_NXP], k4[MPCB_NXP], xt[MPCB_NXP];
        double t = t0 + j * hs, tt;
        plt_f(xc, ul, a, &t, b, k1);
        for (int i = 0; i < MPCB_NXP; ++i) xt[i] = xc[i] + 0.5 * hs * k1[i];
        tt = t + 0.5 * hs;
        plt_f(xt, ul, a, &tt, b, k2);
        for (int i = 0; i < MPCB_NXP; ++i) xt[i] = xc[i] + 0.5 * hs * k2[i];
        plt_f(xt, ul, a, &tt, b, k3);
        for (int i = 0; i < MPCB_NXP; ++i) xt[i] = xc[i] + hs * k3[i];
        tt = t + hs;
        plt_f(xt, ul, a, &tt, b, k4);
        for (int i = 0; i < MPCB_NXP; ++i) xc[i] += (hs / 6.0) * (k1[i] + 2.0 * k2[i] + 2.0 * k3[i] + k4[i]);
    }
    double post[MPCB_NXP];
    plt_post(a, b, post);
    for (int i = 0; i < MPCB_NXP; ++i) x[i] = xc[i] + post[i];
#else
    double xn[MPCB_NXP];
    plt_F(xc, ul, a, &t0, b, xn);
    for (int i = 0; i < MPCB_NXP; ++i) x[i] = xn[i];
#endif
}
#endif
```

Baseline: 739,700.

## Solve target IPM with a lane group per instance using shared-memory workspace

```diff
diff --git a/mpc-code_b200/csrc/mpcb_api.cu b/mpc-code_b200/csrc/mpcb_api.cu
--- a/mpc-code_b200/csrc/mpcb_api.cu
+++ b/mpc-code_b200/csrc/mpcb_api.cu
@@ -188,17 +188,26 @@
 #endif
 
 #if MPCB_HAS_TARGET
-__global__ void __launch_bounds__(64) k_target(int B, const double* par, double* w, double* f, int* status, int* iters,
-                                               TgtShared S) {
-    const int inst = blockIdx.x * blockDim.x + threadIdx.x;
+#define TGT_WS_BYTES ((int)sizeof(double) * TgtWs::total)
+#define TGT_IPB_MAX (MPCB_TGT_BLOCK > MPCB_TGT_LANES ? MPCB_TGT_BLOCK / MPCB_TGT_LANES : 1)
+#define TGT_IPB (TGT_IPB_MAX * TGT_WS_BYTES <= 227 * 1024 ? TGT_IPB_MAX : (TGT_WS_BYTES <= 227 * 1024 ? 227 * 1024 / TGT_WS_BYTES : 1))
+#define TGT_THREADS (TGT_IPB * MPCB_TGT_LANES)
+#define TGT_SMEM_BYTES (TGT_IPB * TGT_WS_BYTES)
+__global__ void __launch_bounds__(TGT_THREADS) k_target(int B, const double* par, double* w, double* f, int* status, int* iters,
+                                                        TgtShared S) {
+    extern __shared__ __align__(16) double tgt_smem[];
+    const int g = threadIdx.x / MPCB_TGT_LANES, inst = blockIdx.x * TGT_IPB + g;
     if (inst >= B) return;
-    tgt_solve_regular(par + (size_t)inst * MPCB_NPARSS, w + (size_t)inst * NWS, f + inst, status + inst, iters + inst, S);
-}
-__global__ void __launch_bounds__(64) k_target_resto(int B, const double* par, double* w, double* f, int* status, int* iters,
-                                                     TgtShared S) {
-    const int inst = blockIdx.x * blockDim.x + threadIdx.x;
+    tgt_solve_regular(par + (size_t)inst * MPCB_NPARSS, w + (size_t)inst * NWS, f + inst, status + inst, iters + inst, S,
+                      tgt_smem + (size_t)g * TgtWs::total);
+}
+__global__ void __launch_bounds__(TGT_THREADS) k_target_resto(int B, const double* par, double* w, double* f, int* status, int* iters,
+                                                              TgtShared S) {
+    extern __shared__ __align__(16) double tgt_smem[];
+    const int g = threadIdx.x / MPCB_TGT_LANES, inst = blockIdx.x * TGT_IPB + g;
     if (inst >= B) return;
-    tgt_solve_resto(par + (size_t)inst * MPCB_NPARSS, w + (size_t)inst * NWS, f + inst, status + inst, iters + inst, S);
+    tgt_solve_resto(par + (size_t)inst * MPCB_NPARSS, w + (size_t)inst * NWS, f + inst, status + inst, iters + inst, S,
+                    tgt_smem + (size_t)g * TgtWs::total);
 }
 #endif
 
@@ -503,6 +512,10 @@
     h->ss_lbx = h->ss_ubx = nullptr;
 #if MPCB_HAS_TARGET
     CK(cudaMalloc(&h->ss_lbx, sizeof(double) * NWS)); CK(cudaMalloc(&h->ss_ubx, sizeof(double) * NWS));
+    if (TGT_SMEM_BYTES > 48 * 1024) {
+        CK(cudaFuncSetAttribute(k_target, cudaFuncAttributeMaxDynamicSharedMemorySize, (int)TGT_SMEM_BYTES));
+        CK(cudaFuncSetAttribute(k_target_resto, cudaFuncAttributeMaxDynamicSharedMemorySize, (int)TGT_SMEM_BYTES));
+    }
 #endif
     CK(cudaMalloc(&h->Qkf, sizeof(double) * NXI * NXI)); CK(cudaMalloc(&h->Rkf, sizeof(double) * NY * NY));
     CK(cudaMalloc(&h->Kest, sizeof(double) * NXI * NY));
@@ -799,9 +812,9 @@
 int mpcb_target(mpcb_handle_t h, const double* par_ss, double* wss, double* fss, int* status, int* iters, void* stream) {
 #if MPCB_HAS_TARGET
     TgtShared S; S.lbx = h->ss_lbx; S.ubx = h->ss_ubx; S.o = to_ipm(h->opts_ss);
-    { Prof p(h, (cudaStream_t)stream, KC_TARGET); k_target<<<nblk(h->B, MPCB_TGT_BLOCK), MPCB_TGT_BLOCK, 0, (cudaStream_t)stream>>>(h->B, par_ss, wss, fss, status, iters, S); }
+    { Prof p(h, (cudaStream_t)stream, KC_TARGET); k_target<<<nblk(h->B, TGT_IPB), TGT_THREADS, TGT_SMEM_BYTES, (cudaStream_t)stream>>>(h->B, par_ss, wss, fss, status, iters, S); }
 #if !MPCB_DENSE_SH
-    { Prof p(h, (cudaStream_t)stream, KC_TARGET); k_target_resto<<<nblk(h->B, MPCB_TGT_BLOCK), MPCB_TGT_BLOCK, 0, (cudaStream_t)stream>>>(h->B, par_ss, wss, fss, status, iters, S); }
+    { Prof p(h, (cudaStream_t)stream, KC_TARGET); k_target_resto<<<nblk(h->B, TGT_IPB), TGT_THREADS, TGT_SMEM_BYTES, (cudaStream_t)stream>>>(h->B, par_ss, wss, fss, status, iters, S); }
     h->host_launches += 1;
 #endif
     CK(cudaGetLastError());
diff --git a/mpc-code_b200/csrc/mpcb_target.cuh b/mpc-code_b200/csrc/mpcb_target.cuh
--- a/mpc-code_b200/csrc/mpcb_target.cuh
+++ b/mpc-code_b200/csrc/mpcb_target.cuh
@@ -16,46 +16,86 @@
 #define NKS  (NVT + MCS)
 #define NWSP (NWS * (NWS + 1) / 2)
 
+#ifndef MPCB_TGT_LANES
+#define MPCB_TGT_LANES 4
+#endif
+#if defined(__CUDA_ARCH__) && (MPCB_TGT_LANES > 1)
+#  define T_LANE        ((int)(threadIdx.x & (MPCB_TGT_LANES - 1)))
+#  define T_NL          MPCB_TGT_LANES
+#  define T_BASE        ((int)(threadIdx.x & 31) & ~(MPCB_TGT_LANES - 1))
+#  define T_MASK        (MPCB_TGT_LANES == 32 ? 0xffffffffu : (((1u << (MPCB_TGT_LANES & 31)) - 1u) << T_BASE))
+#  define T_SYNC()      __syncwarp(T_MASK)
+#  define T_MAX(v)      group_max<MPCB_TGT_LANES>(v, T_MASK)
+#  define T_MIN(v)      group_min<MPCB_TGT_LANES>(v, T_MASK)
+#  define T_BCAST(v, l) __shfl_sync(T_MASK, v, l, MPCB_TGT_LANES)
+#  define T_FIRST(p)    (__ffs(__ballot_sync(T_MASK, p) >> T_BASE) - 1)
+__device__ __forceinline__ void t_argmax(double& v, int& i) {
+MPCB_UNROLL
+    for (int o = MPCB_TGT_LANES / 2; o > 0; o >>= 1) {
+        const double ov = __shfl_xor_sync(T_MASK, v, o, MPCB_TGT_LANES);
+        const int oi = __shfl_xor_sync(T_MASK, i, o, MPCB_TGT_LANES);
+        if (ov > v || (ov == v && oi < i)) { v = ov; i = oi; }
+    }
+}
+#else
+#  define T_LANE        0
+#  define T_NL          1
+#  define T_SYNC()
+#  define T_MAX(v)      (v)
+#  define T_MIN(v)      (v)
+#  define T_BCAST(v, l) (v)
+#  define T_FIRST(p)    ((p) ? 0 : -1)
+MPCB_HD void t_argmax(double&, int&) {}
+#endif
+
 template <int N>
 MPCB_HD void bk_factor(double* A, int* ipiv, int* npos, int* nneg, int* nzero) {
     const double alpha = (1.0 + sqrt(17.0)) / 8.0;
+    const int lane = T_LANE;
     *npos = *nneg = *nzero = 0;
     int k = 0;
     while (k < N) {
         int kstep = 1, kp = k;
         const double absakk = fabs(A[k + N * k]);
         int imax = k; double colmax = 0.0;
-        for (int i = k + 1; i < N; ++i) { const double v = fabs(A[i + N * k]); if (v > colmax) { colmax = v; imax = i; } }
+        for (int i = k + 1 + lane; i < N; i += T_NL) { const double v = fabs(A[i + N * k]); if (v > colmax) { colmax = v; imax = i; } }
+        t_argmax(colmax, imax);
         if (fmax(absakk, colmax) == 0.0) {
-            *nzero += 1; ipiv[k] = k + 1; k += 1; continue;
+            *nzero += 1; if (lane == 0) ipiv[k] = k + 1; k += 1; continue;
         }
         if (absakk >= alpha * colmax) {
             kp = k;
         } else {
             double rowmax = 0.0;
-            for (int j = k; j < imax; ++j) rowmax = fmax(rowmax, fabs(A[imax + N * j]));
-            for (int i = imax + 1; i < N; ++i) rowmax = fmax(rowmax, fabs(A[i + N * imax]));
+            for (int j = k + lane; j < imax; j += T_NL) rowmax = fmax(rowmax, fabs(A[imax + N * j]));
+            for (int i = imax + 1 + lane; i < N; i += T_NL) rowmax = fmax(rowmax, fabs(A[i + N * imax]));
+            rowmax = T_MAX(rowmax);
             if (absakk >= alpha * colmax * (colmax / rowmax)) kp = k;
             else if (fabs(A[imax + N * imax]) >= alpha * rowmax) kp = imax;
             else { kp = imax; kstep = 2; }
         }
         const int kk = k + kstep - 1;
         if (kp != kk) {
-            for (int i = kp + 1; i < N; ++i) { const double t = A[i + N * kk]; A[i + N * kk] = A[i + N * kp]; A[i + N * kp] = t; }
-            for (int j = kk + 1; j < kp; ++j) { const double t = A[j + N * kk]; A[j + N * kk] = A[kp + N * j]; A[kp + N * j] = t; }
-            { const double t = A[kk + N * kk]; A[kk + N * kk] = A[kp + N * kp]; A[kp + N * kp] = t; }
-            if (kstep == 2) { const double t = A[k + 1 + N * k]; A[k + 1 + N * k] = A[kp + N * k]; A[kp + N * k] = t; }
+            T_SYNC();
+            for (int i = kp + 1 + lane; i < N; i += T_NL) { const double t = A[i + N * kk]; A[i + N * kk] = A[i + N * kp]; A[i + N * kp] = t; }
+            for (int j = kk + 1 + lane; j < kp; j += T_NL) { const double t = A[j + N * kk]; A[j + N * kk] = A[kp + N * j]; A[kp + N * j] = t; }
+            if (lane == 0) {
+                { const double t = A[kk + N * kk]; A[kk + N * kk] = A[kp + N * kp]; A[kp + N * kp] = t; }
+                if (kstep == 2) { const double t = A[k + 1 + N * k]; A[k + 1 + N * k] = A[kp + N * k]; A[kp + N * k] = t; }
+            }
+            T_SYNC();
         }
         if (kstep == 1) {
             const double dkk = A[k + N * k];
             if (dkk > 0.0) *npos += 1; else if (dkk < 0.0) *nneg += 1; else *nzero += 1;
             const double r1 = 1.0 / dkk;
-            for (int j = k + 1; j < N; ++j) {
+            for (int j = k + 1 + lane; j < N; j += T_NL) {
                 const double ajk = A[j + N * k] * r1;
                 for (int i = j; i < N; ++i) A[i + N * j] -= A[i + N * k] * ajk;
             }
-            for (int i = k + 1; i < N; ++i) A[i + N * k] *= r1;
-            ipiv[k] = kp + 1;
+            T_SYNC();
+            for (int i = k + 1 + lane; i < N; i += T_NL) A[i + N * k] *= r1;
+            if (lane == 0) ipiv[k] = kp + 1;
         } else {
             const double a = A[k + N * k], b = A[k + 1 + N * k], c = A[k + 1 + N * (k + 1)];
             const double det = a * c - b * b;
@@ -67,65 +107,110 @@
                 const double d11 = c / d21, d22 = a / d21;
                 const double t = 1.0 / (d11 * d22 - 1.0);
                 d21 = t / d21;
-                for (int j = k + 2; j < N; ++j) {
+                for (int j = k + 2 + lane; j < N; j += T_NL) {
                     const double wk = d21 * (d11 * A[j + N * k] - A[j + N * (k + 1)]);
                     const double wkp1 = d21 * (d22 * A[j + N * (k + 1)] - A[j + N * k]);
                     for (int i = j; i < N; ++i) A[i + N * j] -= A[i + N * k] * wk + A[i + N * (k + 1)] * wkp1;
+                }
+                T_SYNC();
+                for (int j = k + 2 + lane; j < N; j += T_NL) {
+                    const double wk = d21 * (d11 * A[j + N * k] - A[j + N * (k + 1)]);
+                    const double wkp1 = d21 * (d22 * A[j + N * (k + 1)] - A[j + N * k]);
                     A[j + N * k] = wk;
                     A[j + N * (k + 1)] = wkp1;
                 }
             }
-            ipiv[k] = -(kp + 1); ipiv[k + 1] = -(kp + 1);
-        }
+            if (lane == 0) { ipiv[k] = -(kp + 1); ipiv[k + 1] = -(kp + 1); }
+        }
+        T_SYNC();
         k += kstep;
     }
 }
 
 template <int N>
 MPCB_HD void bk_solve(const double* A, const int* ipiv, double* b) {
+    const int lane = T_LANE;
     int k = 0;
     while (k < N) {
         if (ipiv[k] > 0) {
             const int kp = ipiv[k] - 1;
-            if (kp != k) { const double t = b[k]; b[k] = b[kp]; b[kp] = t; }
-            for (int i = k + 1; i < N; ++i) b[i] -= b[k] * A[i + N * k];
-            b[k] /= A[k + N * k];
+            const double bk = b[kp], bkp = b[k];
+            T_SYNC();
+            for (int i = k + 1 + lane; i < N; i += T_NL) { const double bi = (i == kp) ? bkp : b[i]; b[i] = bi - bk * A[i + N * k]; }
+            if (lane == 0) b[k] = bk / A[k + N * k];
             k += 1;
         } else {
             const int kp = -ipiv[k] - 1;
-            if (kp != k + 1) { const double t = b[k + 1]; b[k + 1] = b[kp]; b[kp] = t; }
-            for (int i = k + 2; i < N; ++i) b[i] -= b[k] * A[i + N * k] + b[k + 1] * A[i + N * (k + 1)];
-            const double akm1k = A[k + 1 + N * k];
-            const double akm1 = A[k + N * k] / akm1k, ak = A[k + 1 + N * (k + 1)] / akm1k;
-            const double denom = akm1 * ak - 1.0;
-            const double bkm1 = b[k] / akm1k, bk = b[k + 1] / akm1k;
-            b[k] = (ak * bkm1 - bk) / denom;
-            b[k + 1] = (akm1 * bk - bkm1) / denom;
+            const double bk = b[k], bk1 = b[kp], bkp = b[k + 1];
+            T_SYNC();
+            for (int i = k + 2 + lane; i < N; i += T_NL) {
+                const double bi = (i == kp) ? bkp : b[i];
+                b[i] = bi - (bk * A[i + N * k] + bk1 * A[i + N * (k + 1)]);
+            }
+            if (lane == 0) {
+                const double akm1k = A[k + 1 + N * k];
+                const double akm1 = A[k + N * k] / akm1k, ak = A[k + 1 + N * (k + 1)] / akm1k;
+                const double denom = akm1 * ak - 1.0;
+                const double bkm1 = bk / akm1k, bkk = bk1 / akm1k;
+                b[k] = (ak * bkm1 - bkk) / denom;
+                b[k + 1] = (akm1 * bkk - bkm1) / denom;
+            }
             k += 2;
         }
-    }
-    k = N - 1;
-    while (k >= 0) {
-        if (ipiv[k] > 0) {
-            double a = b[k];
-            for (int i = k + 1; i < N; ++i) a -= A[i + N * k] * b[i];
-            b[k] = a;
-            const int kp = ipiv[k] - 1;
-            if (kp != k) { const double t = b[k]; b[k] = b[kp]; b[kp] = t; }
-            k -= 1;
-        } else {
-            double a = b[k], a1 = b[k - 1];
-            for (int i = k + 1; i < N; ++i) { a -= A[i + N * k] * b[i]; a1 -= A[i + N * (k - 1)] * b[i]; }
-            b[k] = a; b[k - 1] = a1;
-            const int kp = -ipiv[k] - 1;
-            if (kp != k) { const double t = b[k]; b[k] = b[kp]; b[kp] = t; }
-            k -= 2;
-        }
-    }
+        T_SYNC();
+    }
+    if (lane == 0) {
+        k = N - 1;
+        while (k >= 0) {
+            if (ipiv[k] > 0) {
+                double a = b[k];
+                for (int i = k + 1; i < N; ++i) a -= A[i + N * k] * b[i];
+                b[k] = a;
+                const int kp = ipiv[k] - 1;
+                if (kp != k) { const double t = b[k]; b[k] = b[kp]; b[kp] = t; }
+                k -= 1;
+            } else {
+                double a = b[k], a1 = b[k - 1];
+                for (int i = k + 1; i < N; ++i) { a -= A[i + N * k] * b[i]; a1 -= A[i + N * (k - 1)] * b[i]; }
+                b[k] = a; b[k - 1] = a1;
+                const int kp = -ipiv[k] - 1;
+                if (kp != k) { const double t = b[k]; b[k] = b[kp]; b[kp] = t; }
+                k -= 2;
+            }
+        }
+    }
+    T_SYNC();
 }
 
 #if MPCB_HAS_TARGET
 struct TgtShared { const double *lbx, *ubx; IpmOpts o; };
+
+#define TPAD(n) (((n) + 1) / 2 * 2)
+struct TgtWs {
+    static constexpr int K = 0;
+    static constexpr int rhs = K + TPAD(NKS * NKS);
+    static constexpr int J = rhs + TPAD(NKS);
+    static constexpr int Hp = J + TPAD(MCS * NVT);
+    static constexpr int grad = Hp + TPAD(NWSP);
+    static constexpr int c = grad + TPAD(NVT);
+    static constexpr int y = c + TPAD(MCS);
+    static constexpr int w = y + TPAD(MCS);
+    static constexpr int lo = w + TPAD(NVT);
+    static constexpr int hi = lo + TPAD(NVT);
+    static constexpr int zL = hi + TPAD(NVT);
+    static constexpr int zU = zL + TPAD(NVT);
+    static constexpr int dzL = zU + TPAD(NVT);
+    static constexpr int dzU = dzL + TPAD(NVT);
+    static constexpr int qL = dzU + TPAD(NVT);
+    static constexpr int qU = qL + TPAD(NVT);
+    static constexpr int gL = qU + TPAD(NVT);
+    static constexpr int gU = gL + TPAD(NVT);
+    static constexpr int filt = gU + TPAD(NVT);
+    static constexpr int f = filt + 2 * MPCB_MAXFILT;
+    static constexpr int wt = f + 2;
+    static constexpr int ipiv = wt + MPCB_TGT_LANES * TPAD(NVT);
+    static constexpr int total = ipiv + TPAD((NKS + 2 * NVT + 1) / 2);
+};
 
 MPCB_HD void tgt_eval(const double* w, const double* par, const double* lam, bool derivs,
                       double* f, double* c, double* grad, double* J , double* Hp ) {
@@ -168,37 +253,52 @@
 
 #define TGT_NEEDS_RESTO 1000
 template <bool MPCB_TGT_RESTO>
-MPCB_HD void tgt_solve_t(const double* par, double* w_io, double* fout, int* status_out, int* iters_out, const TgtShared& S) {
+MPCB_HD void tgt_solve_t(const double* par, double* w_io, double* fout, int* status_out, int* iters_out, const TgtShared& S,
+                         double* ws) {
     const IpmOpts& o = S.o;
     const double rf = o.bound_relax;
-    double w[NVT], lo[NVT], hi[NVT]; bool hl[NVT], hu[NVT];
-    int nb = 0;
-    for (int i = 0; i < NWS; ++i) {
+    const int lane = T_LANE;
+    double *K = ws + TgtWs::K, *rhs = ws + TgtWs::rhs, *J = ws + TgtWs::J, *Hp = ws + TgtWs::Hp, *grad = ws + TgtWs::grad;
+    double *c = ws + TgtWs::c, *y = ws + TgtWs::y, *w = ws + TgtWs::w, *lo = ws + TgtWs::lo, *hi = ws + TgtWs::hi;
+    double *zL = ws + TgtWs::zL, *zU = ws + TgtWs::zU, *dzL = ws + TgtWs::dzL, *dzU = ws + TgtWs::dzU;
+    double *qL = ws + TgtWs::qL, *qU = ws + TgtWs::qU, *gL = ws + TgtWs::gL, *gU = ws + TgtWs::gU, *filt = ws + TgtWs::filt;
+    double* wt = ws + TgtWs::wt + lane * TPAD(NVT);
+    int* ipiv = reinterpret_cast<int*>(ws + TgtWs::ipiv);
+    int* hl = ipiv + NKS;
+    int* hu = hl + NVT;
+    for (int i = lane; i < NWS; i += T_NL) {
         hl[i] = fin(S.lbx[i]); hu[i] = fin(S.ubx[i]);
         lo[i] = hl[i] ? rlo(S.lbx[i], rf) : S.lbx[i];
         hi[i] = hu[i] ? rhi(S.ubx[i], rf) : S.ubx[i];
-        nb += (hl[i] ? 1 : 0) + (hu[i] ? 1 : 0);
         w[i] = push_in(w_io[i], lo[i], hi[i], o.bound_push);
     }
     if (NGT > 0) {
-        double f0, c0[MCS];
-        for (int i = NWS; i < NVT; ++i) w[i] = 0.0;
-        tgt_eval(w, par, nullptr, false, &f0, c0, nullptr, nullptr, nullptr);
-        for (int i = NWS; i < NVT; ++i) {
-            hl[i] = false; hu[i] = true; lo[i] = -INFINITY; hi[i] = rhi(0.0, rf); nb += 1;
-            w[i] = push_in(c0[NX + NY + (i - NWS)], lo[i], hi[i], o.bound_push);
-        }
-    }
-    double y[MCS], zL[NVT], zU[NVT];
-    for (int i = 0; i < MCS; ++i) y[i] = 0.0;
-    for (int i = 0; i < NVT; ++i) { zL[i] = hl[i] ? 1.0 : 0.0; zU[i] = hu[i] ? 1.0 : 0.0; }
+        for (int i = NWS + lane; i < NVT; i += T_NL) w[i] = 0.0;
+        T_SYNC();
+        if (lane == 0) tgt_eval(w, par, nullptr, false, ws + TgtWs::f, c, nullptr, nullptr, nullptr);
+        T_SYNC();
+        for (int i = NWS + lane; i < NVT; i += T_NL) {
+            hl[i] = 0; hu[i] = 1; lo[i] = -INFINITY; hi[i] = rhi(0.0, rf);
+            w[i] = push_in(c[NX + NY + (i - NWS)], lo[i], hi[i], o.bound_push);
+        }
+    }
+    for (int i = lane; i < MCS; i += T_NL) y[i] = 0.0;
+    for (int i = lane; i < NVT; i += T_NL) { zL[i] = hl[i] ? 1.0 : 0.0; zU[i] = hu[i] ? 1.0 : 0.0; }
+    T_SYNC();
+    int nb = 0;
+    for (int i = 0; i < NVT; ++i) nb += hl[i] + hu[i];
     double mu = o.mu_init, tau = fmax(0.99, 1.0 - mu), dw_last = 0.0, theta0 = -1.0;
-    double filt[2 * MPCB_MAXFILT]; int nfilt = 0, acc = 0, it = 0, status = -1;
+    int nfilt = 0, acc = 0, it = 0, status = -1;
     bool resto = false; int resto_calls = 0; double theta_entry = 0.0;
-    double f = 0.0, c[MCS], grad[NVT], J[MCS * NVT], Hp[NWSP];
+    double f = 0.0;
     bool evaluate = true;
     while (true) {
-        if (evaluate) tgt_eval(w, par, y, true, &f, c, grad, J, Hp);
+        if (evaluate) {
+            T_SYNC();
+            if (lane == 0) tgt_eval(w, par, y, true, ws + TgtWs::f, c, grad, J, Hp);
+            T_SYNC();
+            f = ws[TgtWs::f];
+        }
         evaluate = false;
         if (it == 0 && !resto) {
             double chk = f;
@@ -207,14 +307,15 @@
             if (!(chk == chk) || !fin(chk)) { status = -13; break; }
         }
         double dual = 0.0, prim = 0.0, ysum = 0.0, zsum = 0.0, c0 = 0.0;
-        for (int j = 0; j < NVT; ++j) {
+        for (int j = lane; j < NVT; j += T_NL) {
             double r = grad[j] - zL[j] + zU[j];
             for (int i = 0; i < MCS; ++i) r += J[i + MCS * j] * y[i];
             dual = fmax(dual, fabs(r));
-            zsum += zL[j] + zU[j];
             if (hl[j]) c0 = fmax(c0, fabs((w[j] - lo[j]) * zL[j]));
             if (hu[j]) c0 = fmax(c0, fabs((hi[j] - w[j]) * zU[j]));
         }
+        dual = T_MAX(dual); c0 = T_MAX(c0);
+        for (int j = 0; j < NVT; ++j) zsum += zL[j] + zU[j];
         for (int i = 0; i < MCS; ++i) { prim = fmax(prim, fabs(c[i])); ysum += fabs(y[i]); }
         const double sd = fmax(100.0, (ysum + zsum) / (double)(MCS + nb > 0 ? MCS + nb : 1)) / 100.0;
         const double sc = fmax(100.0, zsum / (double)(nb > 0 ? nb : 1)) / 100.0;
@@ -231,21 +332,24 @@
         bool changed = false;
         while (!resto && mu > mu_min) {
             double cm = 0.0;
-            for (int j = 0; j < NVT; ++j) {
+            for (int j = lane; j < NVT; j += T_NL) {
                 if (hl[j]) cm = fmax(cm, fabs((w[j] - lo[j]) * zL[j] - mu));
                 if (hu[j]) cm = fmax(cm, fabs((hi[j] - w[j]) * zU[j] - mu));
             }
+            cm = T_MAX(cm);
             if (fmax(fmax(dual / sd, prim), cm / sc) > 10.0 * mu) break;
             mu = fmax(mu_min, fmin(0.2 * mu, pow(mu, 1.5)));
             changed = true;
         }
         if (changed) { tau = fmax(0.99, 1.0 - mu); nfilt = 0; }
-        double K[NKS * NKS], rhs[NKS]; int ipiv[NKS];
         double dwreg = 0.0, dcreg = 0.0; bool first = true, ok = false;
         for (int attempt = 0; attempt < 60; ++attempt) {
-            for (int i = 0; i < NKS * NKS; ++i) K[i] = 0.0;
-            for (int j = 0; j < NVT; ++j) {
-                if (j < NWS) for (int i = j; i < NWS; ++i) K[i + NKS * j] = resto ? 0.0 : Hp[tri(i, j)];
+            T_SYNC();
+            for (int j = lane; j < NKS; j += T_NL) {
+                double* Kj = K + NKS * j;
+                for (int i = 0; i < NKS; ++i) Kj[i] = 0.0;
+                if (j >= NVT) { Kj[j] = -dcreg; continue; }
+                if (j < NWS) for (int i = j; i < NWS; ++i) Kj[i] = resto ? 0.0 : Hp[tri(i, j)];
                 double sig = dwreg;
                 if (resto) {
                     const double sc = fmax(1.0, fabs(w[j]));
@@ -256,10 +360,10 @@
                     if (hl[j]) sig += zL[j] / (w[j] - lo[j]);
                     if (hu[j]) sig += zU[j] / (hi[j] - w[j]);
                 }
-                K[j + NKS * j] += sig;
-                for (int i = 0; i < MCS; ++i) K[NVT + i + NKS * j] = J[i + MCS * j];
-            }
-            for (int i = 0; i < MCS; ++i) K[NVT + i + NKS * (NVT + i)] = -dcreg;
+                Kj[j] += sig;
+                for (int i = 0; i < MCS; ++i) Kj[NVT + i] = J[i + MCS * j];
+            }
+            T_SYNC();
             int np_, nn_, nz_;
             bk_factor<NKS>(K, ipiv, &np_, &nn_, &nz_);
             if (np_ == NVT && nn_ == MCS && nz_ == 0) { ok = true; break; }
@@ -270,7 +374,7 @@
         }
         if (!ok) { status = -3; break; }
         if (dwreg > 0.0) dw_last = dwreg;
-        for (int j = 0; j < NVT; ++j) {
+        for (int j = lane; j < NVT; j += T_NL) {
             double r = grad[j];
             for (int i = 0; i < MCS; ++i) r += J[i + MCS * j] * y[i];
             if (resto) r = 0.0;
@@ -278,28 +382,35 @@
             if (hu[j]) r += mu / (hi[j] - w[j]);
             rhs[j] = -r;
         }
-        for (int i = 0; i < MCS; ++i) rhs[NVT + i] = -c[i];
+        for (int i = lane; i < MCS; i += T_NL) rhs[NVT + i] = -c[i];
+        T_SYNC();
         bk_solve<NKS>(K, ipiv, rhs);
         double amax = 1.0, az = 1.0, gphid = 0.0, barr = 0.0, theta = 0.0;
-        double dzL[NVT], dzU[NVT];
+        for (int j = lane; j < NVT; j += T_NL) {
+            const double dv = rhs[j];
+            dzL[j] = dzU[j] = 0.0;
+            if (hl[j]) {
+                const double dl = w[j] - lo[j];
+                gL[j] = log(dl); qL[j] = mu / dl;
+                if (dv < 0.0) amax = fmin(amax, -tau * dl / dv);
+                dzL[j] = mu / dl - zL[j] - zL[j] / dl * dv;
+                if (dzL[j] < 0.0) az = fmin(az, -tau * zL[j] / dzL[j]);
+            }
+            if (hu[j]) {
+                const double du = hi[j] - w[j];
+                gU[j] = log(du); qU[j] = mu / du;
+                if (dv > 0.0) amax = fmin(amax, tau * du / dv);
+                dzU[j] = mu / du - zU[j] + zU[j] / du * dv;
+                if (dzU[j] < 0.0) az = fmin(az, -tau * zU[j] / dzU[j]);
+            }
+        }
+        amax = T_MIN(amax); az = T_MIN(az);
+        T_SYNC();
         for (int j = 0; j < NVT; ++j) {
             const double dv = rhs[j];
             gphid += grad[j] * dv;
-            dzL[j] = dzU[j] = 0.0;
-            if (hl[j]) {
-                const double dl = w[j] - lo[j];
-                barr += log(dl); gphid -= mu / dl * dv;
-                if (dv < 0.0) amax = fmin(amax, -tau * dl / dv);
-                dzL[j] = mu / dl - zL[j] - zL[j] / dl * dv;
-                if (dzL[j] < 0.0) az = fmin(az, -tau * zL[j] / dzL[j]);
-            }
-            if (hu[j]) {
-                const double du = hi[j] - w[j];
-                barr += log(du); gphid += mu / du * dv;
-                if (dv > 0.0) amax = fmin(amax, tau * du / dv);
-                dzU[j] = mu / du - zU[j] + zU[j] / du * dv;
-                if (dzU[j] < 0.0) az = fmin(az, -tau * zU[j] / dzU[j]);
-            }
+            if (hl[j]) { barr += gL[j]; gphid -= qL[j] * dv; }
+            if (hu[j]) { barr += gU[j]; gphid += qU[j] * dv; }
         }
         for (int i = 0; i < MCS; ++i) theta += fabs(c[i]);
         const double phi = f - mu * barr;
@@ -311,25 +422,38 @@
         else amin = 1e-5;
         amin *= 0.05;
         double alpha = amax; bool accepted = false, ftype = false;
-        double wt[NVT], ft, ct[MCS];
+        int la = -1;
         if (MPCB_TGT_RESTO && resto) {
-            double th_t = 0.0;
-            while (alpha > 1e-5) {
-                for (int j = 0; j < NVT; ++j) wt[j] = w[j] + alpha * rhs[j];
-                tgt_eval(wt, par, y, false, &ft, ct, nullptr, nullptr, nullptr);
-                th_t = 0.0;
-                for (int i = 0; i < MCS; ++i) th_t += fabs(ct[i]);
-                if ((th_t == th_t) && fin(th_t) && th_t <= (1.0 - 1e-4 * alpha) * theta) { accepted = true; break; }
-                alpha *= 0.5;
+            double ft = 0.0, th_t = 0.0;
+            while (true) {
+                double a = alpha;
+                for (int l = 0; l < lane; ++l) a *= 0.5;
+                bool pass = false; double ft_l = 0.0, th_l = 0.0;
+                if (a > 1e-5) {
+                    for (int j = 0; j < NVT; ++j) wt[j] = w[j] + a * rhs[j];
+                    double ct[MCS];
+                    tgt_eval(wt, par, y, false, &ft_l, ct, nullptr, nullptr, nullptr);
+                    for (int i = 0; i < MCS; ++i) th_l += fabs(ct[i]);
+                    pass = (th_l == th_l) && fin(th_l) && th_l <= (1.0 - 1e-4 * a) * theta;
+                }
+                la = T_FIRST(pass);
+                if (la >= 0) { alpha = T_BCAST(a, la); ft = T_BCAST(ft_l, la); th_t = T_BCAST(th_l, la); accepted = true; break; }
+                const double alast = T_BCAST(a, T_NL - 1);
+                if (!(alast > 1e-5)) break;
+                alpha = alast * 0.5;
             }
             if (!accepted) { status = theta > 1e-4 ? 2 : -2; break; }
+            T_SYNC();
+            const double* wa = ws + TgtWs::wt + la * TPAD(NVT);
+            for (int j = lane; j < NVT; j += T_NL) {
+                w[j] = wa[j];
+                if (hl[j]) { const double d = w[j] - lo[j]; zL[j] = mu / d; gL[j] = log(d); }
+                if (hu[j]) { const double d = hi[j] - w[j]; zU[j] = mu / d; gU[j] = log(d); }
+            }
+            for (int i = lane; i < MCS; i += T_NL) y[i] = 0.0;
+            T_SYNC();
             double b_t = 0.0;
-            for (int j = 0; j < NVT; ++j) {
-                w[j] = wt[j];
-                if (hl[j]) { const double d = w[j] - lo[j]; zL[j] = mu / d; b_t += log(d); }
-                if (hu[j]) { const double d = hi[j] - w[j]; zU[j] = mu / d; b_t += log(d); }
-            }
-            for (int i = 0; i < MCS; ++i) y[i] = 0.0;
+            for (int j = 0; j < NVT; ++j) { if (hl[j]) b_t += gL[j]; if (hu[j]) b_t += gU[j]; }
             const double ph_t = ft - mu * b_t;
             bool leave = th_t <= 0.9 * theta_entry;
             if (leave) for (int i = 0; i < nfilt; ++i) if (th_t >= filt[2 * i] && ph_t >= filt[2 * i + 1]) { leave = false; break; }
@@ -338,67 +462,87 @@
             evaluate = true;
             continue;
         }
-        while (alpha >= amin * (1.0 - 1e-12) && alpha > 1e-16) {
-            for (int j = 0; j < NVT; ++j) wt[j] = w[j] + alpha * rhs[j];
-            tgt_eval(wt, par, y, false, &ft, ct, nullptr, nullptr, nullptr);
-            double th_t = 0.0, b_t = 0.0;
-            for (int i = 0; i < MCS; ++i) th_t += fabs(ct[i]);
-            for (int j = 0; j < NVT; ++j) { if (hl[j]) b_t += log(wt[j] - lo[j]); if (hu[j]) b_t += log(hi[j] - wt[j]); }
-            const double ph_t = ft - mu * b_t;
-            bool okk = (th_t == th_t) && (ph_t == ph_t) && fin(th_t) && fin(ph_t) && th_t <= theta_max;
-            if (okk) for (int i = 0; i < nfilt; ++i) if (th_t >= filt[2 * i] && ph_t >= filt[2 * i + 1]) { okk = false; break; }
-            if (okk) {
-                const bool sw = gphid < 0.0 && theta <= theta_min && alpha * pow(-gphid, 2.3) > pow(theta, 1.1);
-                const double eps = 10.0 * 2.220446049250313e-16 * fabs(phi);
-                if (sw) { if (ph_t - phi - eps <= 1e-8 * alpha * gphid) { accepted = true; ftype = true; } }
-                else if (th_t <= (1.0 - 1e-5) * theta || ph_t - eps <= phi - 1e-8 * theta) accepted = true;
-            }
-            if (accepted) break;
-            alpha *= 0.5;
+        while (true) {
+            double a = alpha;
+            for (int l = 0; l < lane; ++l) a *= 0.5;
+            bool pass = false, ftype_l = false;
+            if (a >= amin * (1.0 - 1e-12) && a > 1e-16) {
+                for (int j = 0; j < NVT; ++j) wt[j] = w[j] + a * rhs[j];
+                double ft, ct[MCS];
+                tgt_eval(wt, par, y, false, &ft, ct, nullptr, nullptr, nullptr);
+                double th_t = 0.0, b_t = 0.0;
+                for (int i = 0; i < MCS; ++i) th_t += fabs(ct[i]);
+                for (int j = 0; j < NVT; ++j) { if (hl[j]) b_t += log(wt[j] - lo[j]); if (hu[j]) b_t += log(hi[j] - wt[j]); }
+                const double ph_t = ft - mu * b_t;
+                bool okk = (th_t == th_t) && (ph_t == ph_t) && fin(th_t) && fin(ph_t) && th_t <= theta_max;
+                if (okk) for (int i = 0; i < nfilt; ++i) if (th_t >= filt[2 * i] && ph_t >= filt[2 * i + 1]) { okk = false; break; }
+                if (okk) {
+                    const bool sw = gphid < 0.0 && theta <= theta_min && a * pow(-gphid, 2.3) > pow(theta, 1.1);
+                    const double eps = 10.0 * 2.220446049250313e-16 * fabs(phi);
+                    if (sw) { if (ph_t - phi - eps <= 1e-8 * a * gphid) { pass = true; ftype_l = true; } }
+                    else if (th_t <= (1.0 - 1e-5) * theta || ph_t - eps <= phi - 1e-8 * theta) pass = true;
+                }
+            }
+            la = T_FIRST(pass);
+            if (la >= 0) { alpha = T_BCAST(a, la); ftype = T_BCAST((int)ftype_l, la) != 0; accepted = true; break; }
+            const double alast = T_BCAST(a, T_NL - 1);
+            if (!(alast >= amin * (1.0 - 1e-12) && alast > 1e-16)) break;
+            alpha = alast * 0.5;
         }
         if (!accepted) {
             if (theta < 1e-6 || resto_calls >= 3) { status = theta > 1e-4 ? 2 : -2; break; }
             if (!MPCB_TGT_RESTO) { status = TGT_NEEDS_RESTO; break; }
-            if (nfilt < MPCB_MAXFILT) { filt[2 * nfilt] = (1.0 - 1e-5) * theta; filt[2 * nfilt + 1] = phi - 1e-8 * theta; nfilt++; }
+            if (nfilt < MPCB_MAXFILT) {
+                if (lane == 0) { filt[2 * nfilt] = (1.0 - 1e-5) * theta; filt[2 * nfilt + 1] = phi - 1e-8 * theta; }
+                nfilt++;
+            }
             resto = true; resto_calls += 1; theta_entry = theta;
             continue;
         }
-        if (!ftype && nfilt < MPCB_MAXFILT) { filt[2 * nfilt] = (1.0 - 1e-5) * theta; filt[2 * nfilt + 1] = phi - 1e-8 * theta; nfilt++; }
-        for (int j = 0; j < NVT; ++j) {
-            w[j] = wt[j];
+        if (!ftype && nfilt < MPCB_MAXFILT) {
+            if (lane == 0) { filt[2 * nfilt] = (1.0 - 1e-5) * theta; filt[2 * nfilt + 1] = phi - 1e-8 * theta; }
+            nfilt++;
+        }
+        T_SYNC();
+        const double* wa = ws + TgtWs::wt + la * TPAD(NVT);
+        for (int j = lane; j < NVT; j += T_NL) {
+            w[j] = wa[j];
             if (hl[j]) { const double dn = w[j] - lo[j]; zL[j] = fmax(fmin(zL[j] + az * dzL[j], 1e10 * mu / dn), mu / (1e10 * dn)); }
             if (hu[j]) { const double dn = hi[j] - w[j]; zU[j] = fmax(fmin(zU[j] + az * dzU[j], 1e10 * mu / dn), mu / (1e10 * dn)); }
         }
-        for (int i = 0; i < MCS; ++i) y[i] += alpha * rhs[NVT + i];
+        for (int i = lane; i < MCS; i += T_NL) y[i] += alpha * rhs[NVT + i];
         it += 1;
         evaluate = true;
     }
+    T_SYNC();
     if (o.honor_original_bounds) {
-        for (int j = 0; j < NWS; ++j) w[j] = fmin(fmax(w[j], S.lbx[j]), S.ubx[j]);
-        double ct[MCS];
-        tgt_eval(w, par, y, false, &f, ct, nullptr, nullptr, nullptr);
-    }
-    for (int j = 0; j < NWS; ++j) w_io[j] = w[j];
-    *fout = f; *status_out = status; *iters_out = it;
-}
-
-MPCB_HD void tgt_solve_regular(const double* par, double* w, double* fout, int* status_out, int* iters_out, const TgtShared& S) {
+        for (int j = lane; j < NWS; j += T_NL) w[j] = fmin(fmax(w[j], S.lbx[j]), S.ubx[j]);
+        T_SYNC();
+        if (lane == 0) { double ct[MCS]; tgt_eval(w, par, y, false, ws + TgtWs::f, ct, nullptr, nullptr, nullptr); }
+        T_SYNC();
+        f = ws[TgtWs::f];
+    }
+    if (status != TGT_NEEDS_RESTO)
+        for (int j = lane; j < NWS; j += T_NL) w_io[j] = w[j];
+    if (lane == 0) { *fout = f; *status_out = status; *iters_out = it; }
+}
+
+MPCB_HD void tgt_solve_regular(const double* par, double* w, double* fout, int* status_out, int* iters_out, const TgtShared& S,
+                               double* ws) {
 #if MPCB_DENSE_SH
-    tgt_solve_t<true>(par, w, fout, status_out, iters_out, S);
+    tgt_solve_t<true>(par, w, fout, status_out, iters_out, S, ws);
 #else
-    double w0[NWS];
-    for (int i = 0; i < NWS; ++i) w0[i] = w[i];
-    tgt_solve_t<false>(par, w, fout, status_out, iters_out, S);
-    if (*status_out == TGT_NEEDS_RESTO)
-        for (int i = 0; i < NWS; ++i) w[i] = w0[i];
-#endif
-}
-MPCB_HD void tgt_solve_resto(const double* par, double* w, double* fout, int* status_out, int* iters_out, const TgtShared& S) {
-    if (*status_out == TGT_NEEDS_RESTO) tgt_solve_t<true>(par, w, fout, status_out, iters_out, S);
+    tgt_solve_t<false>(par, w, fout, status_out, iters_out, S, ws);
+#endif
+}
+MPCB_HD void tgt_solve_resto(const double* par, double* w, double* fout, int* status_out, int* iters_out, const TgtShared& S,
+                             double* ws) {
+    if (*status_out == TGT_NEEDS_RESTO) tgt_solve_t<true>(par, w, fout, status_out, iters_out, S, ws);
 }
 MPCB_HD void tgt_solve(const double* par, double* w, double* fout, int* status_out, int* iters_out, const TgtShared& S) {
-    tgt_solve_regular(par, w, fout, status_out, iters_out, S);
-    tgt_solve_resto(par, w, fout, status_out, iters_out, S);
+    double ws[TgtWs::total];
+    tgt_solve_regular(par, w, fout, status_out, iters_out, S, ws);
+    tgt_solve_resto(par, w, fout, status_out, iters_out, S, ws);
 }
 #endif
 
```

Result: faster. 758,500, median of 6 (+2.5%).
